# EmanuelOverflow/LSTM-TensorSpark

Measured on NVIDIA H100. Metric: samples/sec, higher is better.
Workload: dtype bf16

## Files before the change

### lstm_tensorspark_b200/csrc/bindings.cpp

```cpp
#include <torch/extension.h>
#include <ATen/cuda/CUDAContext.h>
#include <c10/cuda/CUDAGuard.h>
#include <c10/cuda/CUDAException.h>
#include <cuda_runtime.h>

#include <cmath>
#include <optional>
#include <string>
#include <vector>

using torch::Tensor;

extern "C" {
int ts_lstm_pointwise_fwd(const void*, const float*, const float*, void*, float*, void*, int, int, int, cudaStream_t, const void*,
                          const int*, int);
int ts_transpose01_rows(const void*, void*, int, int, long long, cudaStream_t);
int ts_lstm_seq_cluster_probe(int);
int ts_lstm_seq_config(int, int, int, int, int*);
int ts_transpose2d_b16(const void*, void*, int, int, cudaStream_t);
int ts_colsum_bf16(const void*, float*, void*, int, int, int, int, int, int, cudaStream_t);
long long ts_colsum_scratch_bytes(int, int);
int ts_lstm_pointwise_bwd(const void*, const float*, const float*, const void*, const float*, const float*, void*,
                          float*, int, int, int, cudaStream_t, const int*, int, float*);
int ts_xent_rows(const float*, const long long*, float*, float*, int*, int, int, cudaStream_t);
int ts_flat_adam(float*, const float*, float*, float*, void*, long long, float, float, float, float, float, float,
                 cudaStream_t, int*, long long, const float*);
int ts_flat_sgd(float*, const float*, void*, long long, float, float, float, cudaStream_t, long long, const float*);
long long ts_flat_grad_norm_scratch(long long);
int ts_flat_grad_norm(const float*, const float*, long long, float, float, long long, float, double*, float*, cudaStream_t);
int ts_cast_bf16(const float*, void*, long long, cudaStream_t);
int ts_fused_allreduce(const unsigned long long*, unsigned long long, unsigned long long, unsigned long long, float*,
                       float*, unsigned int*, int*, long long, int, int, int, int, int, int, float, float, float, float,
                       float, double, cudaStream_t, int*, long long, int, int);
int ts_ar_bump_step(int*, cudaStream_t);
int ts_ar_max_blocks();
int ts_ar_flag_words();
int ts_ar_slots();
int ts_head_fwd_tc(const void*, int, const float*, const float*, const long long*, float*, float*, float*, int*, int, int, int, cudaStream_t);
int ts_head_logits_generic(const void*, const float*, const float*, float*, int, int, int, int, cudaStream_t);
int ts_head_bwd(const void*, const float*, const float*, const float*, void*, float*, float*, int, int, int, int, int, cudaStream_t);
int ts_head_step_fwd_generic_parts(int);
int ts_head_step_fwd(const void*, int, int, const float*, const float*, const long long*, const int*, float*, float*, float*, int*,
                     unsigned int*, float*, int*, int*, int, int, int, int, int*, cudaStream_t);
long long ts_head_step_bwd_scratch(int, int, int);
int ts_head_step_bwd_tickets(int);
int ts_head_step_bwd(const void*, const float*, const float*, const float*, void*, float*, float*, float*, unsigned int*, int, int, int,
                     int, int, cudaStream_t);
int ts_vocab_head_parts(int);
int ts_vocab_head_blocks(int);
int ts_vocab_head_fwd(const void*, const void*, int, const float*, const long long*, const int*, void*, float*, float*, int*, unsigned int*,
                      float*, int*, int*, int, int, int, int, int, cudaStream_t);
int ts_vocab_head_dlogits(const void*, const void*, int, const float*, const long long*, const int*, const float*, const float*, const int*,
                          void*, int, int, int, int, int, int, int, cudaStream_t);
int ts_vocab_head_colsum(const void*, float*, int, int, int, cudaStream_t);
int ts_vocab_sample(const void*, const void*, int, const float*, float, unsigned int, int*, const int*, void*, int*, unsigned int*, int*,
                    float*, int*, float*, int, int, int, int, int, int, cudaStream_t);
int ts_vocab_sample_logits(const float*, const float*, float, unsigned int, int*, const int*, void*, int*, unsigned int*, int*, float*, int*,
                           float*, int, int, int, int, cudaStream_t);
int ts_vocab_head_logits(const void*, const void*, int, const float*, float*, int, int, int, int, cudaStream_t);
int ts_vocab_threshold(const float*, int, int, int, double, float, float*, cudaStream_t);
int ts_gemm_generic(const void*, const void*, void*, const float*, int, int, int, long long, long long, long long, long long, long long,
                    int, int, int, float, cudaStream_t);
int ts_gemm2(const void*, const void*, void*, const float*, int, int, int, int, int, int, int, int, int, int, int, int, int,
             const unsigned int*, const int*, unsigned int*, int*, int, int, int, int, float*, int, cudaStream_t);
int ts_lstm_seq_fwd(const void*, const void*, const float*, const void*, const float*, void*, const float*, void*, void*, int,
                    int, int, unsigned int*, int, cudaStream_t, const void*, const unsigned int*, int, int, int, const int*, int,
                    void*, const int*, const unsigned int*);
int ts_lstm_seq_bwd(const void*, const void*, const void*, const float*, const void*, float*, float*, void*, void*, int,
                    int, int, unsigned int*, int, cudaStream_t, const unsigned int*, int, int, int, const int*, int,
                    const int*, const unsigned int*);
int ts_dropout(const void*, void*, int, int, int, int, int, const int*, const unsigned int*, cudaStream_t);
int ts_lstm_seq_prologue(const void*, const float*, void*, float*, void*, unsigned int*, int, int, cudaStream_t);
int ts_seq_pool_fwd(const void*, int, const int*, const float*, int, int, int, int, float*, int*, cudaStream_t);
int ts_seq_pool_attn_scores(float*, const float*, const float*, const int*, int, int, int, float*, cudaStream_t);
int ts_seq_pool_attn_bwd(const void*, int, const float*, const float*, const float*, const float*, const int*, int, int, int, int,
                         float*, void*, float*, unsigned int*, float*, float*, int, int, cudaStream_t);
int ts_seq_pool_bwd(const float*, const int*, const int*, const float*, const float*, int, int, int, int, void*, int, cudaStream_t);
void ts_embed_scratch_numel(long long, long long, long long, long long*);
int ts_embed_fwd(const void*, int, const int*, const int*, int, int, int, int, void*, cudaStream_t);
int ts_embed_bwd(const void*, int, const int*, const int*, int, int, int, int, float*, int, int*, int*, float*, cudaStream_t);
int ts_embed_bwd_launches();
const char* ts_last_error();
}

namespace {

void check(int rc, const char* what) {
  if (rc != 0) {
    std::string msg = std::string(what) + " failed: rc=" + std::to_string(rc);
    if (rc > 0) msg += std::string(" (") + cudaGetErrorString((cudaError_t)rc) + ")";
    const char* le = ts_last_error();
    if (le && le[0]) msg += std::string(" [") + le + "]";
    TORCH_CHECK(false, msg);
  }
}
cudaStream_t stream() { return at::cuda::getCurrentCUDAStream().stream(); }
void chk_cuda(const Tensor& t, const char* n) {
  TORCH_CHECK(t.is_cuda(), n, " must be a CUDA tensor");
  TORCH_CHECK(t.is_contiguous(), n, " must be contiguous");
}
int is_bf16(const Tensor& t) {
  TORCH_CHECK(t.scalar_type() == torch::kBFloat16 || t.scalar_type() == torch::kFloat32, "dtype must be bf16 or fp32");
  return t.scalar_type() == torch::kBFloat16 ? 1 : 0;
}
const float* fptr(const std::optional<Tensor>& t) { return t.has_value() ? t->data_ptr<float>() : nullptr; }
const int* lengths_ptr(const std::optional<Tensor>& lengths, int64_t B, const Tensor& like) {
  if (!lengths.has_value()) return nullptr;
  const Tensor& l = *lengths;
  TORCH_CHECK(l.is_cuda() && l.device() == like.device(), "lengths must be on the batch's device");
  TORCH_CHECK(l.scalar_type() == torch::kInt32, "lengths must be int32");
  TORCH_CHECK(l.dim() == 1 && l.size(0) == B, "lengths must be [B] (B = ", B, ")");
  TORCH_CHECK(l.is_contiguous(), "lengths must be contiguous");
  return l.data_ptr<int>();
}
const int* drop_args(const std::optional<Tensor>& step, const std::vector<int64_t>& desc, const Tensor& like, unsigned int (&out)[5]) {
  if (!step.has_value()) return nullptr;
  TORCH_CHECK(step->is_cuda() && step->device() == like.device() && step->scalar_type() == torch::kInt32 && step->numel() == 1,
              "dropout: the step counter must be an int32 [1] tensor on the batch's device");
  TORCH_CHECK(desc.size() == 5, "dropout: desc = {key0, key1, thr, c2, row0}");
  TORCH_CHECK(desc[2] >= 1 && desc[2] <= 65535 && desc[4] >= 0, "dropout: thr in [1, 65535], row0 >= 0");
  for (int i = 0; i < 5; ++i) out[i] = (unsigned int)(uint32_t)desc[i];
  return step->data_ptr<int>();
}

int direction_flag(bool reverse, const std::optional<Tensor>& in_gate, bool extra_signal) {
  TORCH_CHECK(!reverse || (!in_gate.has_value() && !extra_signal), "reverse: the layer wavefront (in_gate / extra_signal) is forward-only");
  return reverse ? 1 : 0;
}

Tensor transpose01(const Tensor& x) {
  chk_cuda(x, "x");
  TORCH_CHECK(x.dim() == 3 && x.is_contiguous(), "transpose01: expected a contiguous [B,T,D] tensor");
  c10::cuda::CUDAGuard g(x.device());
  const int B = x.size(0), T = x.size(1);
  const long long row_bytes = (long long)x.size(2) * x.element_size();
  TORCH_CHECK(row_bytes % 16 == 0, "transpose01: row size must be a multiple of 16 bytes");
  auto out = torch::empty({x.size(1), x.size(0), x.size(2)}, x.options());
  check(ts_transpose01_rows(x.data_ptr(), out.data_ptr(), B, T, row_bytes, stream()), "transpose01");
  return out;
}

Tensor transpose2d(const Tensor& x) {
  chk_cuda(x, "x");
  TORCH_CHECK(x.dim() == 2 && x.is_contiguous() && x.element_size() == 2, "transpose2d: expected a contiguous 2-D 16-bit tensor");
  c10::cuda::CUDAGuard g(x.device());
  auto out = torch::empty({x.size(1), x.size(0)}, x.options());
  check(ts_transpose2d_b16(x.data_ptr(), out.data_ptr(), (int)x.size(0), (int)x.size(1), stream()), "transpose2d");
  return out;
}

void* colsum_scratch(const Tensor& x) {
  static std::vector<Tensor> bufs(64);
  const int dev = x.device().index();
  const int64_t need = ts_colsum_scratch_bytes((int)x.size(0), (int)x.size(1));
  if (!bufs[dev].defined() || bufs[dev].numel() < need)
    bufs[dev] = torch::zeros({need}, torch::TensorOptions().device(x.device()).dtype(torch::kUInt8));
  return bufs[dev].data_ptr();
}

Tensor colsum_bf16(const Tensor& x) {
  chk_cuda(x, "x");
  TORCH_CHECK(x.dim() == 2 && x.is_contiguous() && is_bf16(x) && x.size(1) % 256 == 0, "colsum_bf16: contiguous bf16 [rows, cols], cols % 256 == 0");
  c10::cuda::CUDAGuard g(x.device());
  auto out = torch::empty({x.size(1)}, x.options().dtype(torch::kFloat32));
  check(ts_colsum_bf16(x.data_ptr(), out.data_ptr<float>(), colsum_scratch(x), (int)x.size(0), (int)x.size(1), (int)x.size(1), 0, 0, 0, stream()), "colsum_bf16");
  return out;
}

void colsum_bf16_into(const Tensor& x, Tensor out, bool overwrite, bool pdl, int64_t col0, int64_t ncols, int64_t max_ctas) {
  chk_cuda(x, "x"); chk_cuda(out, "out");
  TORCH_CHECK(x.dim() == 2 && is_bf16(x) && x.size(1) % 256 == 0 && out.scalar_type() == torch::kFloat32 && out.numel() == x.size(1),
              "colsum_bf16_into: bf16 [rows, cols % 256 == 0] -> fp32 [cols]");
  if (ncols <= 0) { col0 = 0; ncols = x.size(1); }
  TORCH_CHECK(col0 % 256 == 0 && ncols % 256 == 0 && col0 + ncols <= x.size(1), "colsum_bf16_into: 256-aligned column range");
  c10::cuda::CUDAGuard g(x.device());
  check(ts_colsum_bf16((const char*)x.data_ptr() + 2 * col0, out.data_ptr<float>() + col0, colsum_scratch(x), (int)x.size(0), (int)ncols,
                       (int)x.size(1), overwrite ? 0 : 1, pdl ? 1 : 0, (int)max_ctas, stream()), "colsum_bf16_into");
}

std::vector<Tensor> lstm_pointwise_fwd(const Tensor& pre, const Tensor& bias, const Tensor& c_prev, const std::optional<Tensor>& h_prev,
                                       const std::optional<Tensor>& lengths, int64_t t) {
  chk_cuda(pre, "pre"); chk_cuda(bias, "bias"); chk_cuda(c_prev, "c_prev");
  c10::cuda::CUDAGuard g(pre.device());
  int B = pre.size(0), H = pre.size(1) / 4;
  TORCH_CHECK(bias.scalar_type() == torch::kFloat32 && c_prev.scalar_type() == torch::kFloat32, "bias/c must be fp32");
  TORCH_CHECK(c_prev.numel() == (int64_t)B * H && bias.numel() == 4 * H, "shape mismatch");
  const int* lp = lengths_ptr(lengths, B, pre);
  if (lp) {
    TORCH_CHECK(h_prev.has_value(), "lstm_pointwise_fwd: lengths need h_prev");
    chk_cuda(*h_prev, "h_prev");
    TORCH_CHECK(h_prev->scalar_type() == pre.scalar_type() && h_prev->numel() == (int64_t)B * H, "h_prev: [B,H] in pre's dtype");
  }
  auto h = torch::empty({B, H}, pre.options());
  auto c = torch::empty({B, H}, c_prev.options());
  auto act = torch::empty_like(pre);
  check(ts_lstm_pointwise_fwd(pre.data_ptr(), bias.data_ptr<float>(), c_prev.data_ptr<float>(), h.data_ptr(),
                              c.data_ptr<float>(), act.data_ptr(), B, H, is_bf16(pre), stream(), lp ? h_prev->data_ptr() : nullptr,
                              lp, (int)t), "lstm_pointwise_fwd");
  return {h, c, act};
}

std::vector<Tensor> lstm_pointwise_bwd(const std::optional<Tensor>& dh_a, const std::optional<Tensor>& dh_b,
                                       const std::optional<Tensor>& dc_in, const Tensor& act, const Tensor& c_prev,
                                       const Tensor& c_new, const std::optional<Tensor>& lengths, int64_t t) {
  chk_cuda(act, "act"); chk_cuda(c_prev, "c_prev"); chk_cuda(c_new, "c_new");
  c10::cuda::CUDAGuard g(act.device());
  int B = act.size(0), H = act.size(1) / 4;
  const int* lp = lengths_ptr(lengths, B, act);
  if (dh_a.has_value()) { chk_cuda(*dh_a, "dh_a"); TORCH_CHECK(dh_a->scalar_type() == act.scalar_type(), "dh_a dtype"); }
  if (dh_b.has_value()) { chk_cuda(*dh_b, "dh_b"); TORCH_CHECK(dh_b->scalar_type() == torch::kFloat32, "dh_b fp32"); }
  if (dc_in.has_value()) { chk_cuda(*dc_in, "dc_in"); TORCH_CHECK(dc_in->scalar_type() == torch::kFloat32, "dc fp32"); }
  auto dpre = torch::empty_like(act);
  auto dc = torch::empty_like(c_prev);
  Tensor dh_out = lp ? torch::empty_like(c_prev) : Tensor();
  check(ts_lstm_pointwise_bwd(dh_a.has_value() ? dh_a->data_ptr() : nullptr, fptr(dh_b), fptr(dc_in), act.data_ptr(),
                              c_prev.data_ptr<float>(), c_new.data_ptr<float>(), dpre.data_ptr(), dc.data_ptr<float>(),
                              B, H, is_bf16(act), stream(), lp, (int)t, lp ? dh_out.data_ptr<float>() : nullptr), "lstm_pointwise_bwd");
  if (lp) return {dpre, dc, dh_out};
  return {dpre, dc};
}

Tensor dropout(const Tensor& x, const Tensor& step, const std::vector<int64_t>& desc, int64_t t0) {
  chk_cuda(x, "x");
  TORCH_CHECK(x.dim() >= 2, "dropout: x must be [..., B, H]");
  c10::cuda::CUDAGuard g(x.device());
  unsigned int dd[5];
  const int* ds = drop_args(step, desc, x, dd);
  const int64_t B = x.size(-2), H = x.size(-1), steps = B * H ? x.numel() / (B * H) : 0;
  auto y = torch::empty_like(x);
  check(ts_dropout(x.data_ptr(), y.data_ptr(), (int)steps, (int)B, (int)H, (int)t0, is_bf16(x), ds, dd, stream()), "dropout");
  return y;
}

std::vector<Tensor> xent_rows(const Tensor& logits, const Tensor& labels) {
  chk_cuda(logits, "logits"); chk_cuda(labels, "labels");
  c10::cuda::CUDAGuard g(logits.device());
  TORCH_CHECK(logits.scalar_type() == torch::kFloat32 && labels.scalar_type() == torch::kInt64, "dtypes");
  int B = logits.size(0), C = logits.size(1);
  auto dlogits = torch::empty_like(logits);
  auto loss = torch::zeros({1}, logits.options());
  auto correct = torch::zeros({1}, logits.options().dtype(torch::kInt32));
  check(ts_xent_rows(logits.data_ptr<float>(), (const long long*)labels.data_ptr<int64_t>(), dlogits.data_ptr<float>(),
                     loss.data_ptr<float>(), correct.data_ptr<int>(), B, C, stream()), "xent_rows");
  return {dlogits, loss, correct};
}

std::vector<Tensor> head_fwd(const Tensor& h, const Tensor& W, const Tensor& bias, const Tensor& labels) {
  TORCH_CHECK(h.is_cuda() && h.dim() == 2 && h.stride(1) == 1, "head_fwd: h [B,H] with unit inner stride");
  chk_cuda(W, "W"); chk_cuda(bias, "bias"); chk_cuda(labels, "labels");
  c10::cuda::CUDAGuard g(h.device());
  const int B = h.size(0), H = h.size(1), C = W.size(1);
  TORCH_CHECK(W.size(0) == H && W.scalar_type() == torch::kFloat32 && bias.scalar_type() == torch::kFloat32, "head W/b");
  TORCH_CHECK(labels.scalar_type() == torch::kInt64 && labels.numel() == B, "labels int64 [B]");
  auto fo = torch::TensorOptions().device(h.device()).dtype(torch::kFloat32);
  auto logits = torch::empty({B, C}, fo), dlogits = torch::empty({B, C}, fo);
  auto loss = torch::zeros({1}, fo);
  auto correct = torch::zeros({1}, fo.dtype(torch::kInt32));
  int rc = -1;
  if (h.scalar_type() == torch::kBFloat16)
    rc = ts_head_fwd_tc(h.data_ptr(), (int)h.stride(0), W.data_ptr<float>(), bias.data_ptr<float>(), (const long long*)labels.data_ptr<int64_t>(),
                        logits.data_ptr<float>(), dlogits.data_ptr<float>(), loss.data_ptr<float>(), correct.data_ptr<int>(), B, H, C, stream());
  if (rc == -1) {
    auto hc = h.contiguous();
    check(ts_head_logits_generic(hc.data_ptr(), W.data_ptr<float>(), bias.data_ptr<float>(), logits.data_ptr<float>(), B, H, C, is_bf16(hc), stream()),
          "head_logits_generic");
    check(ts_xent_rows(logits.data_ptr<float>(), (const long long*)labels.data_ptr<int64_t>(), dlogits.data_ptr<float>(),
                       loss.data_ptr<float>(), correct.data_ptr<int>(), B, C, stream()), "xent_rows");
  } else {
    check(rc, "head_fwd_tc");
  }
  return {logits, dlogits, loss, correct};
}

Tensor head_bwd(const Tensor& h, const Tensor& W, const Tensor& dlogits, const std::optional<Tensor>& dloss, Tensor dW, Tensor db,
                bool accumulate) {
  chk_cuda(h, "h"); chk_cuda(W, "W"); chk_cuda(dlogits, "dlogits"); chk_cuda(dW, "dW"); chk_cuda(db, "db");
  c10::cuda::CUDAGuard g(h.device());
  const int B = h.size(0), H = h.size(1), C = W.size(1);
  TORCH_CHECK(dW.scalar_type() == torch::kFloat32 && db.scalar_type() == torch::kFloat32 && dW.numel() == (int64_t)H * C && db.numel() == C, "head_bwd: dW/db");
  TORCH_CHECK(dlogits.scalar_type() == torch::kFloat32 && dlogits.numel() == (int64_t)B * C, "head_bwd: dlogits fp32 [B,C]");
  auto dh = torch::empty_like(h);
  check(ts_head_bwd(h.data_ptr(), W.data_ptr<float>(), dlogits.data_ptr<float>(), fptr(dloss), dh.data_ptr(), dW.data_ptr<float>(),
                    db.data_ptr<float>(), B, H, C, is_bf16(h), accumulate ? 1 : 0, stream()), "head_bwd");
  return dh;
}

std::vector<Tensor> head_step_fwd(const Tensor& h, const Tensor& W, const Tensor& bias, const Tensor& labels,
                                  const std::optional<Tensor>& lengths, int64_t T) {
  TORCH_CHECK(h.is_cuda() && h.dim() == 2 && h.stride(1) == 1, "head_step_fwd: h [T*B,H] with unit inner stride");
  chk_cuda(W, "W"); chk_cuda(bias, "bias"); chk_cuda(labels, "labels");
  c10::cuda::CUDAGuard g(h.device());
  const int R = h.size(0), H = h.size(1), C = W.size(1);
  TORCH_CHECK(T >= 1 && R % T == 0, "head_step_fwd: rows must be T*B");
  const int B = R / (int)T;
  TORCH_CHECK(W.size(0) == H && W.scalar_type() == torch::kFloat32 && bias.scalar_type() == torch::kFloat32 && bias.numel() == C, "head W/b");
  TORCH_CHECK(labels.scalar_type() == torch::kInt64 && labels.dim() == 2 && labels.size(0) == B && labels.size(1) == T, "labels int64 [B,T]");
  const int* lp = nullptr;
  if (lengths.has_value()) {
    chk_cuda(*lengths, "lengths");
    TORCH_CHECK(lengths->scalar_type() == torch::kInt32 && lengths->numel() == B, "lengths int32 [B]");
    lp = lengths->data_ptr<int>();
  }
  auto fo = torch::TensorOptions().device(h.device()).dtype(torch::kFloat32);
  auto io = fo.dtype(torch::kInt32);
  auto logits = torch::empty({B, (int64_t)T, C}, fo), dlogits = torch::empty({R, C}, fo);
  const int parts = ts_head_step_fwd_generic_parts(R);
  auto part_loss = torch::empty({parts}, fo);
  auto ints = torch::zeros({parts + 4}, io);
  auto loss = torch::empty({1}, fo);
  Tensor hc = h;
  if (h.scalar_type() != torch::kBFloat16 && h.stride(0) != H) hc = h.contiguous();
  int used_tc = 0;
  int rc = ts_head_step_fwd(hc.data_ptr(), (int)hc.stride(0), is_bf16(hc), W.data_ptr<float>(), bias.data_ptr<float>(),
                            (const long long*)labels.data_ptr<int64_t>(), lp, logits.data_ptr<float>(), dlogits.data_ptr<float>(),
                            part_loss.data_ptr<float>(), ints.data_ptr<int>(), (unsigned int*)(ints.data_ptr<int>() + parts),
                            loss.data_ptr<float>(), ints.data_ptr<int>() + parts + 1, ints.data_ptr<int>() + parts + 2, (int)T, B, H, C,
                            &used_tc, stream());
  if (rc == -2) {
    hc = h.contiguous();
    rc = ts_head_step_fwd(hc.data_ptr(), H, 1, W.data_ptr<float>(), bias.data_ptr<float>(), (const long long*)labels.data_ptr<int64_t>(),
                          lp, logits.data_ptr<float>(), dlogits.data_ptr<float>(), part_loss.data_ptr<float>(), ints.data_ptr<int>(),
                          (unsigned int*)(ints.data_ptr<int>() + parts), loss.data_ptr<float>(), ints.data_ptr<int>() + parts + 1,
                          ints.data_ptr<int>() + parts + 2, (int)T, B, H, C, &used_tc, stream());
  }
  check(rc, "head_step_fwd");
  return {logits, dlogits, loss, ints.narrow(0, parts + 1, 1), ints.narrow(0, parts + 2, 1),
          torch::full({1}, used_tc, torch::TensorOptions().dtype(torch::kInt32))};
}

Tensor head_step_bwd(const Tensor& h, const Tensor& W, const Tensor& dlogits, const std::optional<Tensor>& dloss, Tensor dW, Tensor db,
                     bool accumulate) {
  chk_cuda(h, "h"); chk_cuda(W, "W"); chk_cuda(dlogits, "dlogits"); chk_cuda(dW, "dW"); chk_cuda(db, "db");
  c10::cuda::CUDAGuard g(h.device());
  const int R = h.size(0), H = h.size(1), C = W.size(1);
  TORCH_CHECK(dW.scalar_type() == torch::kFloat32 && db.scalar_type() == torch::kFloat32 && dW.numel() == (int64_t)H * C && db.numel() == C, "head_step_bwd: dW/db");
  TORCH_CHECK(dlogits.scalar_type() == torch::kFloat32 && dlogits.numel() == (int64_t)R * C, "head_step_bwd: dlogits fp32 [R,C]");
  auto dh = torch::empty_like(h);
  auto fo = torch::TensorOptions().device(h.device()).dtype(torch::kFloat32);
  auto scratch = torch::empty({std::max<long long>(1, ts_head_step_bwd_scratch(R, H, C))}, fo);
  auto tickets = torch::zeros({ts_head_step_bwd_tickets(H)}, fo.dtype(torch::kInt32));
  check(ts_head_step_bwd(h.data_ptr(), W.data_ptr<float>(), dlogits.data_ptr<float>(), fptr(dloss), dh.data_ptr(), dW.data_ptr<float>(),
                         db.data_ptr<float>(), scratch.data_ptr<float>(), (unsigned int*)tickets.data_ptr<int>(), R, H, C, is_bf16(h),
                         accumulate ? 1 : 0, stream()), "head_step_bwd");
  return dh;
}

int64_t vocab_classes(const Tensor& h, const Tensor& Wb, bool w_kmajor, const char* what) {
  TORCH_CHECK(h.dim() == 2 && Wb.dim() == 2 && h.scalar_type() == torch::kBFloat16 && Wb.scalar_type() == torch::kBFloat16 &&
              Wb.size(w_kmajor ? 1 : 0) == h.size(1), what, ": h bf16 [rows,H], Wb bf16 ", w_kmajor ? "[C,H]" : "[H,C]");
  TORCH_CHECK(!w_kmajor || (Wb.is_contiguous() && (uintptr_t)Wb.data_ptr() % 16 == 0), what, ": the table [C,H] must be packed and "
              "16-byte aligned (TMA)");
  return Wb.size(w_kmajor ? 0 : 1);
}

void vocab_head_check(const Tensor& h, const Tensor& Wb, bool w_kmajor, const Tensor& bias, const Tensor& labels, int64_t T) {
  chk_cuda(h, "h"); chk_cuda(Wb, "Wb"); chk_cuda(bias, "bias"); chk_cuda(labels, "labels");
  const int64_t R = h.size(0), H = h.size(1), C = vocab_classes(h, Wb, w_kmajor, "vocab head");
  TORCH_CHECK(H % 64 == 0 && C % 8 == 0 && C >= 8, "vocab head: H % 64 == 0 and C % 8 == 0");
  TORCH_CHECK(T >= 1 && R % T == 0 && R * std::max(C, H) < (int64_t(1) << 40) && R < (int64_t(1) << 31), "vocab head: rows must be T*B");
  TORCH_CHECK(bias.scalar_type() == torch::kFloat32 && bias.numel() == C && ((uintptr_t)bias.data_ptr() % 8) == 0, "vocab head: bias fp32 [C]");
  TORCH_CHECK(labels.scalar_type() == torch::kInt64 && labels.dim() == 2 && labels.size(0) == R / T && labels.size(1) == T, "labels int64 [B,T]");
}

std::vector<Tensor> vocab_head_fwd(const Tensor& h, const Tensor& Wb, bool w_kmajor, const Tensor& bias, const Tensor& labels,
                                   const std::optional<Tensor>& lengths, int64_t T, Tensor part) {
  vocab_head_check(h, Wb, w_kmajor, bias, labels, T);
  c10::cuda::CUDAGuard g(h.device());
  const int R = h.size(0), H = h.size(1), C = Wb.size(w_kmajor ? 0 : 1), B = R / (int)T;
  chk_cuda(part, "part");
  TORCH_CHECK(part.scalar_type() == torch::kFloat32 && part.numel() >= (int64_t)R * ts_vocab_head_parts(C) * 4 &&
              ((uintptr_t)part.data_ptr() % 16) == 0, "vocab head: part scratch");
  auto fo = torch::TensorOptions().device(h.device()).dtype(torch::kFloat32);
  const int blocks = ts_vocab_head_blocks(R);
  auto lse = torch::empty({R}, fo), part_loss = torch::empty({blocks}, fo), loss = torch::empty({1}, fo);
  auto ints = torch::zeros({blocks + 4}, fo.dtype(torch::kInt32));
  int* ip = ints.data_ptr<int>();
  check(ts_vocab_head_fwd(h.data_ptr(), Wb.data_ptr(), w_kmajor ? 1 : 0, bias.data_ptr<float>(), (const long long*)labels.data_ptr<int64_t>(),
                          lengths_ptr(lengths, B, h), part.data_ptr(), lse.data_ptr<float>(), part_loss.data_ptr<float>(), ip,
                          (unsigned int*)(ip + blocks), loss.data_ptr<float>(), ip + blocks + 1, ip + blocks + 2, (int)T, B, H, C,
                          h.get_device(), stream()), "vocab_head_fwd");
  return {lse, loss, ints.narrow(0, blocks + 1, 1), ints.narrow(0, blocks + 2, 1)};
}

void vocab_head_dlogits(const Tensor& h, const Tensor& Wb, bool w_kmajor, const Tensor& bias, const Tensor& labels,
                        const std::optional<Tensor>& lengths, int64_t T, const Tensor& lse, const Tensor& count, const Tensor& dloss,
                        int64_t row0, int64_t rows, Tensor dl) {
  vocab_head_check(h, Wb, w_kmajor, bias, labels, T);
  c10::cuda::CUDAGuard g(h.device());
  const int R = h.size(0), H = h.size(1), C = Wb.size(w_kmajor ? 0 : 1), B = R / (int)T;
  chk_cuda(lse, "lse"); chk_cuda(count, "count"); chk_cuda(dloss, "dloss"); chk_cuda(dl, "dl");
  TORCH_CHECK(lse.scalar_type() == torch::kFloat32 && lse.numel() == R && count.scalar_type() == torch::kInt32 && count.numel() == 1 &&
              dloss.scalar_type() == torch::kFloat32 && dloss.numel() == 1, "vocab head: lse fp32 [R], count int32 [1], dloss fp32 [1]");
  TORCH_CHECK(rows >= 1 && row0 >= 0 && row0 + rows <= R && dl.scalar_type() == torch::kBFloat16 && dl.numel() >= rows * C,
              "vocab head: dl bf16 [rows, C]");
  check(ts_vocab_head_dlogits(h.data_ptr(), Wb.data_ptr(), w_kmajor ? 1 : 0, bias.data_ptr<float>(), (const long long*)labels.data_ptr<int64_t>(),
                              lengths_ptr(lengths, B, h), lse.data_ptr<float>(), dloss.data_ptr<float>(), count.data_ptr<int>(),
                              dl.data_ptr(), (int)T, B, H, C, (int)row0, (int)rows, h.get_device(), stream()), "vocab_head_dlogits");
}

void vocab_head_colsum(const Tensor& dl, Tensor db, bool accumulate) {
  chk_cuda(dl, "dl"); chk_cuda(db, "db");
  c10::cuda::CUDAGuard g(dl.device());
  TORCH_CHECK(dl.dim() == 2 && dl.scalar_type() == torch::kBFloat16 && dl.size(1) % 2 == 0 && db.scalar_type() == torch::kFloat32 &&
              db.numel() == dl.size(1), "vocab head: dl bf16 [rows, C], db fp32 [C]");
  check(ts_vocab_head_colsum(dl.data_ptr(), db.data_ptr<float>(), (int)dl.size(0), (int)dl.size(1), accumulate ? 1 : 0, stream()),
        "vocab_head_colsum");
}

struct SampleOut {
  int* rec_tok = nullptr;
  float* rec_lp = nullptr;
  int N = 0;
};
SampleOut sample_check(int64_t B, const Tensor& like, const Tensor& step, const Tensor& row0, const Tensor& tokens,
                       const std::optional<Tensor>& rec_tok, const std::optional<Tensor>& rec_lp, double temperature) {
  chk_cuda(step, "step"); chk_cuda(row0, "row0"); chk_cuda(tokens, "tokens");
  TORCH_CHECK(row0.scalar_type() == torch::kInt32 && row0.numel() == 1 && row0.device() == like.device(), "vocab sample: row0 int32 [1]");
  TORCH_CHECK(std::isfinite(temperature) && temperature >= 0, "vocab sample: temperature must be finite and >= 0");
  TORCH_CHECK(step.scalar_type() == torch::kInt32 && step.numel() == 1 && step.device() == like.device(), "vocab sample: step int32 [1]");
  TORCH_CHECK(tokens.scalar_type() == torch::kInt32 && tokens.numel() == B && tokens.device() == like.device(), "vocab sample: tokens int32 [B]");
  SampleOut o;
  TORCH_CHECK(rec_tok.has_value() == rec_lp.has_value(), "vocab sample: rec_tok and rec_lp go together");
  if (rec_tok.has_value()) {
    chk_cuda(*rec_tok, "rec_tok"); chk_cuda(*rec_lp, "rec_lp");
    TORCH_CHECK(rec_tok->scalar_type() == torch::kInt32 && rec_tok->dim() == 2 && rec_tok->size(0) == B &&
                rec_lp->scalar_type() == torch::kFloat32 && rec_lp->sizes() == rec_tok->sizes() &&
                rec_tok->device() == like.device() && rec_lp->device() == like.device(), "vocab sample: records int32 / fp32 [B, N]");
    o.rec_tok = rec_tok->data_ptr<int>(); o.rec_lp = rec_lp->data_ptr<float>(); o.N = (int)rec_tok->size(1);
  }
  return o;
}

Tensor vocab_sample(const Tensor& h, const Tensor& Wb, bool w_kmajor, const Tensor& bias, double temperature, int64_t seed, Tensor step,
                    const Tensor& row0, Tensor tokens, const std::optional<Tensor>& rec_tok, const std::optional<Tensor>& rec_lp,
                    int64_t s0) {
  chk_cuda(h, "h"); chk_cuda(Wb, "Wb"); chk_cuda(bias, "bias");
  const int64_t Cw = vocab_classes(h, Wb, w_kmajor, "vocab sample");
  TORCH_CHECK(h.size(0) >= 1 && h.size(0) < (int64_t(1) << 24), "vocab sample: h bf16 [B,H] with 1 <= B < 2^24");
  TORCH_CHECK(h.size(1) % 64 == 0 && Cw % 8 == 0 && Cw >= 8, "vocab sample: H % 64 == 0 and C % 8 == 0");
  TORCH_CHECK(bias.scalar_type() == torch::kFloat32 && bias.numel() == Cw && ((uintptr_t)bias.data_ptr() % 8) == 0,
              "vocab sample: bias fp32 [C]");
  c10::cuda::CUDAGuard g(h.device());
  const int B = h.size(0), H = h.size(1), C = (int)Cw;
  const SampleOut o = sample_check(B, h, step, row0, tokens, rec_tok, rec_lp, temperature);
  const int nt = ts_vocab_head_parts(C);
  auto fo = torch::TensorOptions().device(h.device()).dtype(torch::kFloat32);
  auto part = torch::empty({(int64_t)B * nt * 4}, fo), logprob = torch::empty({B}, fo);
  auto part_arg = torch::empty({(int64_t)B * nt}, fo.dtype(torch::kInt32)), ticket = torch::zeros({1}, fo.dtype(torch::kInt32));
  check(ts_vocab_sample(h.data_ptr(), Wb.data_ptr(), w_kmajor ? 1 : 0, bias.data_ptr<float>(), (float)temperature, (unsigned int)(seed & 0xffffffff),
                        step.data_ptr<int>(), row0.data_ptr<int>(), part.data_ptr(), part_arg.data_ptr<int>(), (unsigned int*)ticket.data_ptr<int>(),
                        tokens.data_ptr<int>(), logprob.data_ptr<float>(), o.rec_tok, o.rec_lp, o.N, (int)s0, B, H, C, h.get_device(),
                        stream()), "vocab_sample");
  return logprob;
}

void chk_logits(const Tensor& logits) {
  chk_cuda(logits, "logits");
  TORCH_CHECK(logits.dim() == 2 && logits.scalar_type() == torch::kFloat32 && logits.is_contiguous() && logits.size(0) >= 1 &&
              logits.size(1) >= 1 && logits.size(1) < (int64_t(1) << 31) && logits.numel() < (int64_t(1) << 40),
              "vocab sample: logits fp32 [B, C], packed");
}

Tensor vocab_sample_logits(const Tensor& logits, double temperature, int64_t seed, Tensor step, const Tensor& row0, Tensor tokens,
                           const std::optional<Tensor>& rec_tok, const std::optional<Tensor>& rec_lp, int64_t s0,
                           const std::optional<Tensor>& tau) {
  chk_logits(logits);
  c10::cuda::CUDAGuard g(logits.device());
  const int B = logits.size(0), C = logits.size(1);
  const SampleOut o = sample_check(B, logits, step, row0, tokens, rec_tok, rec_lp, temperature);
  if (tau.has_value()) {
    chk_cuda(*tau, "tau");
    TORCH_CHECK(tau->scalar_type() == torch::kFloat32 && tau->numel() == B && tau->is_contiguous() && tau->device() == logits.device(),
                "vocab sample: tau fp32 [B]");
    TORCH_CHECK(temperature > 0, "vocab sample: a threshold needs temperature > 0 (greedy keeps the arg-max, which no filter drops)");
  }
  const int nt = ts_vocab_head_parts(C);
  auto fo = torch::TensorOptions().device(logits.device()).dtype(torch::kFloat32);
  auto part = torch::empty({(int64_t)B * nt * 4}, fo), logprob = torch::empty({B}, fo);
  auto part_arg = torch::empty({(int64_t)B * nt}, fo.dtype(torch::kInt32)), ticket = torch::zeros({1}, fo.dtype(torch::kInt32));
  check(ts_vocab_sample_logits(logits.data_ptr<float>(), tau.has_value() ? tau->data_ptr<float>() : nullptr, (float)temperature,
                               (unsigned int)(seed & 0xffffffff), step.data_ptr<int>(),
                               row0.data_ptr<int>(), part.data_ptr(), part_arg.data_ptr<int>(), (unsigned int*)ticket.data_ptr<int>(), tokens.data_ptr<int>(),
                               logprob.data_ptr<float>(), o.rec_tok, o.rec_lp, o.N, (int)s0, B, C, stream()), "vocab_sample_logits");
  return logprob;
}

Tensor vocab_head_logits(const Tensor& h, const Tensor& Wb, bool w_kmajor, const Tensor& bias) {
  chk_cuda(h, "h"); chk_cuda(Wb, "Wb"); chk_cuda(bias, "bias");
  const int64_t Cw = vocab_classes(h, Wb, w_kmajor, "vocab logits");
  TORCH_CHECK(h.is_contiguous() && h.size(0) >= 1 && h.size(0) < (int64_t(1) << 24), "vocab logits: h bf16 [B,H] packed, 1 <= B < 2^24");
  TORCH_CHECK(h.size(1) % 64 == 0 && Cw % 8 == 0 && Cw >= 8, "vocab logits: H % 64 == 0 and C % 8 == 0");
  TORCH_CHECK(bias.scalar_type() == torch::kFloat32 && bias.numel() == Cw && ((uintptr_t)bias.data_ptr() % 8) == 0,
              "vocab logits: bias fp32 [C]");
  c10::cuda::CUDAGuard g(h.device());
  const int B = h.size(0), H = h.size(1), C = (int)Cw;
  auto logits = torch::empty({B, C}, torch::TensorOptions().device(h.device()).dtype(torch::kFloat32));
  check(ts_vocab_head_logits(h.data_ptr(), Wb.data_ptr(), w_kmajor ? 1 : 0, bias.data_ptr<float>(), logits.data_ptr<float>(), B, H, C,
                             h.get_device(), stream()), "vocab_head_logits");
  return logits;
}

Tensor vocab_threshold(const Tensor& logits, int64_t top_k, double top_p, double temperature) {
  chk_logits(logits);
  TORCH_CHECK(top_k >= 0, "vocab threshold: top_k must be >= 0 (0 = off), got ", top_k);
  TORCH_CHECK(std::isfinite(top_p) && top_p > 0 && top_p <= 1, "vocab threshold: top_p must be in (0, 1] (1 = off), got ", top_p);
  TORCH_CHECK(std::isfinite(temperature) && temperature > 0, "vocab threshold: temperature must be finite and > 0, got ", temperature);
  c10::cuda::CUDAGuard g(logits.device());
  const int B = logits.size(0), C = logits.size(1);
  auto tau = torch::empty({B}, torch::TensorOptions().device(logits.device()).dtype(torch::kFloat32));
  check(ts_vocab_threshold(logits.data_ptr<float>(), B, C, (int)std::min<int64_t>(top_k, C), top_p, (float)temperature,
                           tau.data_ptr<float>(), stream()), "vocab_threshold");
  return tau;
}

void chk_f32(const Tensor& t, int64_t numel, const char* n) {
  chk_cuda(t, n);
  TORCH_CHECK(t.scalar_type() == torch::kFloat32 && t.numel() == numel, n, ": fp32 with ", numel, " elements");
}

std::vector<Tensor> seq_pool_fwd(const Tensor& h, const std::optional<Tensor>& lengths, int64_t T, int64_t mode,
                                 const std::optional<Tensor>& alpha) {
  chk_cuda(h, "h");
  TORCH_CHECK(h.dim() == 2 && T >= 1 && h.size(0) % T == 0, "seq_pool_fwd: h [T·B, H]");
  TORCH_CHECK(mode >= 0 && mode <= 2, "seq_pool_fwd: mode 0 mean, 1 max, 2 attention");
  c10::cuda::CUDAGuard g(h.device());
  const int B = h.size(0) / T, H = h.size(1);
  if (mode == 2) {
    TORCH_CHECK(alpha.has_value(), "seq_pool_fwd: attention needs alpha");
    chk_f32(*alpha, (int64_t)T * B, "alpha");
  }
  auto fo = h.options().dtype(torch::kFloat32);
  auto s = torch::empty({B, H}, fo);
  auto am = mode == 1 ? torch::empty({B, H}, fo.dtype(torch::kInt32)) : torch::empty({0}, fo.dtype(torch::kInt32));
  check(ts_seq_pool_fwd(h.data_ptr(), is_bf16(h), lengths_ptr(lengths, B, h), fptr(alpha), (int)mode, (int)T, B, H,
                        s.data_ptr<float>(), mode == 1 ? am.data_ptr<int>() : nullptr, stream()), "seq_pool_fwd");
  return {s, am};
}

Tensor seq_pool_attn_scores(Tensor u, const Tensor& ba, const Tensor& v, const std::optional<Tensor>& lengths, int64_t T) {
  chk_cuda(u, "u");
  TORCH_CHECK(u.dim() == 2 && u.scalar_type() == torch::kFloat32 && T >= 1 && u.size(0) % T == 0, "seq_pool_attn_scores: u fp32 [T·B, A]");
  c10::cuda::CUDAGuard g(u.device());
  const int B = u.size(0) / T, A = u.size(1);
  chk_f32(ba, A, "b_a"); chk_f32(v, A, "v");
  auto alpha = torch::empty({T, B}, u.options());
  check(ts_seq_pool_attn_scores(u.data_ptr<float>(), ba.data_ptr<float>(), v.data_ptr<float>(), lengths_ptr(lengths, B, u), (int)T, B, A,
                                alpha.data_ptr<float>(), stream()), "seq_pool_attn_scores");
  return alpha;
}

Tensor seq_pool_attn_bwd(const Tensor& h, const Tensor& ds, const Tensor& alpha, const Tensor& u, const Tensor& v,
                         const std::optional<Tensor>& lengths, int64_t T, Tensor dv, Tensor dba, bool acc_dv, bool acc_dba) {
  chk_cuda(h, "h");
  TORCH_CHECK(h.dim() == 2 && T >= 1 && h.size(0) % T == 0, "seq_pool_attn_bwd: h [T·B, H]");
  c10::cuda::CUDAGuard g(h.device());
  const int B = h.size(0) / T, H = h.size(1), A = u.size(1);
  chk_f32(ds, (int64_t)B * H, "ds"); chk_f32(alpha, (int64_t)T * B, "alpha"); chk_f32(u, (int64_t)T * B * A, "u");
  chk_f32(v, A, "v"); chk_f32(dv, A, "dv"); chk_f32(dba, A, "dba");
  auto fo = h.options().dtype(torch::kFloat32);
  auto dU = torch::empty({h.size(0), A}, h.options());
  auto dalpha = torch::empty({T, B}, fo);
  auto partial = torch::empty({B, 2 * A}, fo);
  auto ticket = torch::zeros({1}, fo.dtype(torch::kInt32));
  check(ts_seq_pool_attn_bwd(h.data_ptr(), is_bf16(h), ds.data_ptr<float>(), alpha.data_ptr<float>(), u.data_ptr<float>(),
                             v.data_ptr<float>(), lengths_ptr(lengths, B, h), (int)T, B, H, A, dalpha.data_ptr<float>(), dU.data_ptr(),
                             partial.data_ptr<float>(), (unsigned int*)ticket.data_ptr<int>(), dv.data_ptr<float>(), dba.data_ptr<float>(),
                             acc_dv ? 1 : 0, acc_dba ? 1 : 0, stream()), "seq_pool_attn_bwd");
  return dU;
}

Tensor seq_pool_bwd(const Tensor& ds, const std::optional<Tensor>& lengths, int64_t T, int64_t mode, const std::optional<Tensor>& argmax,
                    const std::optional<Tensor>& alpha, const std::optional<Tensor>& G, bool out_bf16) {
  chk_cuda(ds, "ds");
  TORCH_CHECK(ds.dim() == 2 && ds.scalar_type() == torch::kFloat32 && T >= 1, "seq_pool_bwd: ds fp32 [B,H]");
  TORCH_CHECK(mode >= 0 && mode <= 2, "seq_pool_bwd: mode 0 mean, 1 max, 2 attention");
  c10::cuda::CUDAGuard g(ds.device());
  const int B = ds.size(0), H = ds.size(1);
  if (mode == 1) {
    TORCH_CHECK(argmax.has_value() && argmax->scalar_type() == torch::kInt32 && argmax->numel() == (int64_t)B * H, "seq_pool_bwd: argmax int32 [B,H]");
    chk_cuda(*argmax, "argmax");
  }
  if (mode == 2) {
    TORCH_CHECK(alpha.has_value() && G.has_value(), "seq_pool_bwd: attention needs alpha and G");
    chk_f32(*alpha, (int64_t)T * B, "alpha"); chk_f32(*G, (int64_t)T * B * H, "G");
  }
  auto dh = torch::empty({T * B, H}, ds.options().dtype(out_bf16 ? torch::kBFloat16 : torch::kFloat32));
  check(ts_seq_pool_bwd(ds.data_ptr<float>(), lengths_ptr(lengths, B, ds), mode == 1 ? argmax->data_ptr<int>() : nullptr, fptr(alpha),
                        fptr(G), (int)mode, (int)T, B, H, dh.data_ptr(), out_bf16 ? 1 : 0, stream()), "seq_pool_bwd");
  return dh;
}

void chk_tokens(const Tensor& tok, const Tensor& like) {
  chk_cuda(tok, "tokens");
  TORCH_CHECK(tok.device() == like.device() && tok.scalar_type() == torch::kInt32 && tok.dim() == 2,
              "tokens must be int32 [B,T] on the table's device");
}

Tensor embed_fwd(const Tensor& table, const Tensor& tokens, const std::optional<Tensor>& lengths) {
  chk_cuda(table, "table");
  TORCH_CHECK(table.dim() == 2, "embed_fwd: table [V,E]");
  chk_tokens(tokens, table);
  c10::cuda::CUDAGuard g(table.device());
  const int B = tokens.size(0), T = tokens.size(1), V = table.size(0), E = table.size(1);
  auto x = torch::empty({T, B, E}, table.options());
  check(ts_embed_fwd(table.data_ptr(), is_bf16(table), tokens.data_ptr<int>(), lengths_ptr(lengths, B, table), T, B, E, V,
                     x.data_ptr(), stream()), "embed_fwd");
  return x;
}

struct EmbedScratch { int* zeroed; int* ints; float* floats; };
EmbedScratch embed_scratch(const Tensor& like, int64_t N, int64_t V, int64_t E) {
  static std::vector<std::vector<Tensor>> bufs(64, std::vector<Tensor>(3));
  static std::vector<Tensor> retired;
  auto& b = bufs[like.device().index()];
  long long need[2];
  ts_embed_scratch_numel(N, V, E, need);
  const int64_t sizes[3] = {2 * V, need[0], need[1]};
  for (int i = 0; i < 3; ++i) {
    if (b[i].defined() && b[i].numel() >= sizes[i]) continue;
    if (b[i].defined()) retired.push_back(b[i]);
    auto opt = torch::TensorOptions().device(like.device()).dtype(i == 2 ? torch::kFloat32 : torch::kInt32);
    b[i] = i == 0 ? torch::zeros({sizes[i]}, opt) : torch::empty({sizes[i]}, opt);
  }
  return {b[0].data_ptr<int>(), b[1].data_ptr<int>(), b[2].data_ptr<float>()};
}

void embed_bwd(const Tensor& dx, const Tensor& tokens, const std::optional<Tensor>& lengths, Tensor dW, bool accumulate) {
  chk_cuda(dx, "dx"); chk_cuda(dW, "dW");
  chk_tokens(tokens, dx);
  const int B = tokens.size(0), T = tokens.size(1);
  TORCH_CHECK(dW.dim() == 2 && dW.scalar_type() == torch::kFloat32 && dW.device() == dx.device(), "embed_bwd: dW fp32 [V,E]");
  const int V = dW.size(0), E = dW.size(1);
  TORCH_CHECK(dx.numel() == (int64_t)T * B * E, "embed_bwd: dx [T·B, E]");
  c10::cuda::CUDAGuard g(dx.device());
  auto s = embed_scratch(dx, (int64_t)T * B, V, E);
  check(ts_embed_bwd(dx.data_ptr(), is_bf16(dx), tokens.data_ptr<int>(), lengths_ptr(lengths, B, dx), T, B, E, V,
                     dW.data_ptr<float>(), accumulate ? 1 : 0, s.zeroed, s.ints, s.floats, stream()), "embed_bwd");
}

const float* clip_ptr(const std::optional<Tensor>& clip, const Tensor& p) {
  if (!clip.has_value()) return nullptr;
  TORCH_CHECK(clip->is_cuda() && clip->device() == p.device() && clip->scalar_type() == torch::kFloat32 && clip->numel() == 2 &&
              clip->is_contiguous(), "clip must be a contiguous fp32 [2] tensor on p's device (flat_grad_norm's out)");
  return clip->data_ptr<float>();
}
void flat_adam(Tensor p, const Tensor& g, Tensor m, Tensor v, std::optional<Tensor> shadow, double lr_t, double b1,
               double b2, double eps, double wd, double gscale, std::optional<Tensor> step_dev, int64_t wd_numel,
               std::optional<Tensor> clip) {
  chk_cuda(p, "p"); chk_cuda(g, "g"); chk_cuda(m, "m"); chk_cuda(v, "v");
  c10::cuda::CUDAGuard gd(p.device());
  TORCH_CHECK(p.numel() == g.numel() && p.numel() == m.numel() && p.numel() == v.numel(), "numel mismatch");
  check(ts_flat_adam(p.data_ptr<float>(), g.data_ptr<float>(), m.data_ptr<float>(), v.data_ptr<float>(),
                     shadow.has_value() ? shadow->data_ptr() : nullptr, p.numel(), lr_t, b1, b2, eps, wd, gscale, stream(),
                     step_dev.has_value() ? step_dev->data_ptr<int>() : nullptr, (long long)wd_numel, clip_ptr(clip, p)),
        "flat_adam");
}
void flat_sgd(Tensor p, const Tensor& g, std::optional<Tensor> shadow, double lr, double wd, double gscale, int64_t wd_numel,
              std::optional<Tensor> clip) {
  chk_cuda(p, "p"); chk_cuda(g, "g");
  c10::cuda::CUDAGuard gd(p.device());
  check(ts_flat_sgd(p.data_ptr<float>(), g.data_ptr<float>(), shadow.has_value() ? shadow->data_ptr() : nullptr,
                    p.numel(), lr, wd, gscale, stream(), (long long)wd_numel, clip_ptr(clip, p)), "flat_sgd");
}
void flat_grad_norm(const Tensor& g, const Tensor& p, Tensor out, Tensor scratch, double max_norm, double wd, double gscale,
                    int64_t wd_numel) {
  chk_cuda(g, "g"); chk_cuda(p, "p"); chk_cuda(out, "out"); chk_cuda(scratch, "scratch");
  c10::cuda::CUDAGuard gd(g.device());
  TORCH_CHECK(g.scalar_type() == torch::kFloat32 && p.scalar_type() == torch::kFloat32 && p.numel() == g.numel(), "flat_grad_norm: g, p fp32 of one size");
  TORCH_CHECK(out.scalar_type() == torch::kFloat32 && out.numel() == 2, "flat_grad_norm: out fp32 [2]");
  TORCH_CHECK(scratch.scalar_type() == torch::kFloat64 && scratch.numel() >= ts_flat_grad_norm_scratch(g.numel()),
              "flat_grad_norm: scratch float64 [flat_grad_norm_scratch(n)]");
  TORCH_CHECK(p.device() == g.device() && out.device() == g.device() && scratch.device() == g.device(), "flat_grad_norm: one device");
  check(ts_flat_grad_norm(g.data_ptr<float>(), p.data_ptr<float>(), g.numel(), wd, gscale, (long long)wd_numel, max_norm,
                          scratch.data_ptr<double>(), out.data_ptr<float>(), stream()), "flat_grad_norm");
}
void cast_bf16(const Tensor& p, Tensor shadow) {
  chk_cuda(p, "p"); chk_cuda(shadow, "shadow");
  c10::cuda::CUDAGuard gd(p.device());
  TORCH_CHECK(shadow.scalar_type() == torch::kBFloat16 && shadow.numel() == p.numel(), "shadow");
  check(ts_cast_bf16(p.data_ptr<float>(), shadow.data_ptr(), p.numel(), stream()), "cast_bf16");
}

void fused_allreduce(const Tensor& ptrs, int64_t mc_in, int64_t mc_param, int64_t mc_shadow, std::optional<Tensor> m,
                     std::optional<Tensor> v, Tensor epochs, Tensor err, int64_t n, int64_t rank, int64_t world,
                     int64_t mode, bool two_shot, bool multicast, int64_t blocks, double lr, double b1, double b2,
                     double eps, double wd, double timeout_s, std::optional<Tensor> step_dev, int64_t wd_numel, bool bump_step, bool pdl) {
  TORCH_CHECK(!ptrs.is_cuda() && ptrs.scalar_type() == torch::kInt64 && ptrs.numel() == 4 * world, "ptrs: cpu int64 [4,world]");
  chk_cuda(epochs, "epochs"); chk_cuda(err, "err");
  c10::cuda::CUDAGuard gd(epochs.device());
  check(ts_fused_allreduce((const unsigned long long*)ptrs.data_ptr<int64_t>(), (unsigned long long)mc_in,
                           (unsigned long long)mc_param, (unsigned long long)mc_shadow,
                           m.has_value() ? m->data_ptr<float>() : nullptr, v.has_value() ? v->data_ptr<float>() : nullptr,
                           (unsigned int*)epochs.data_ptr<int>(), err.data_ptr<int>(), n, (int)rank, (int)world, (int)mode,
                           two_shot ? 1 : 0, multicast ? 1 : 0, (int)blocks, lr, b1, b2, eps, wd, timeout_s, stream(),
                           step_dev.has_value() ? step_dev->data_ptr<int>() : nullptr, (long long)wd_numel, bump_step ? 1 : 0, pdl ? 1 : 0),
        "fused_allreduce");
}

Tensor gemm2(const Tensor& A, const Tensor& B, const std::optional<Tensor>& bias, std::optional<Tensor> out, bool a_mn, bool b_mn,
             bool out_fp32, bool accumulate, int64_t ctas, int64_t bn, int64_t max_ctas, const std::optional<Tensor>& gate,
             const std::vector<int64_t>& gate_cfg, const std::optional<Tensor>& done, const std::optional<Tensor>& gate_err,
             int64_t stream_handle, bool pdl, int64_t a_fold, int64_t b_fold, int64_t fold_cols, const std::optional<Tensor>& rowsum,
             bool rowsum_acc) {
  TORCH_CHECK(A.is_cuda() && B.is_cuda(), "gemm2: CUDA tensors");
  TORCH_CHECK(!(a_fold && b_fold) && (!a_fold || !a_mn) && (!b_fold || b_mn), "gemm2: one folded operand (K-major A or MN-major B)");
  TORCH_CHECK(A.scalar_type() == torch::kBFloat16 && B.scalar_type() == torch::kBFloat16, "gemm2: A/B must be bf16");
  TORCH_CHECK(A.dim() == 2 && B.dim() == 2 && A.stride(1) == 1 && B.stride(1) == 1, "gemm2: 2-D operands with unit inner stride");
  c10::cuda::CUDAGuard gd(A.device());
  if (a_fold) TORCH_CHECK(A.size(0) == a_fold && fold_cols > 0 && A.size(1) % fold_cols == 0, "gemm2: folded A must be [fold, T * fold_cols]");
  if (b_fold) TORCH_CHECK(B.size(0) == b_fold && fold_cols > 0 && B.size(1) % fold_cols == 0, "gemm2: folded B must be [fold, T * fold_cols]");
  const int M = a_fold ? (int)(a_fold * (A.size(1) / fold_cols)) : (a_mn ? A.size(1) : A.size(0));
  const int K = a_fold ? (int)fold_cols : (a_mn ? A.size(0) : A.size(1));
  const int N = b_fold ? (int)fold_cols : (b_mn ? B.size(1) : B.size(0));
  const int Kb = b_fold ? (int)(b_fold * (B.size(1) / fold_cols)) : (b_mn ? B.size(0) : B.size(1));
  TORCH_CHECK(K == Kb, "gemm2: contraction sizes differ (", K, " vs ", Kb, ")");
  Tensor C;
  if (out.has_value()) {
    C = *out;
    TORCH_CHECK(C.is_cuda() && C.dim() == 2 && C.size(0) == M && C.size(1) == N && C.stride(1) == 1, "gemm2: out must be [M,N]");
    TORCH_CHECK(C.scalar_type() == (out_fp32 || accumulate ? torch::kFloat32 : torch::kBFloat16), "gemm2: out dtype");
  } else {
    TORCH_CHECK(!accumulate, "gemm2: accumulate needs out=");
    C = torch::empty({M, N}, A.options().dtype(out_fp32 ? torch::kFloat32 : torch::kBFloat16));
  }
  const int out_mode = accumulate ? 2 : (C.scalar_type() == torch::kFloat32 ? 1 : 0);
  const unsigned int* gp = nullptr;
  int gcfg[7] = {0, 0, 0, 0, 1, 0, 0};
  if (gate.has_value()) {
    TORCH_CHECK(gate->is_cuda() && gate->scalar_type() == torch::kInt32 && gate_cfg.size() == 7, "gemm2: gate int32 cuda + 7 config ints");
    gp = (const unsigned int*)gate->data_ptr<int>();
    for (int i = 0; i < 7; ++i) gcfg[i] = (int)gate_cfg[i];
  }
  float* rp = nullptr;
  if (rowsum.has_value()) {
    TORCH_CHECK(rowsum->is_cuda() && rowsum->scalar_type() == torch::kFloat32 && rowsum->is_contiguous() && rowsum->numel() == M &&
                C.scalar_type() == torch::kFloat32, "gemm2: rowsum must be a contiguous fp32 [M] next to an fp32 output");
    rp = rowsum->data_ptr<float>();
  }
  TORCH_CHECK((ctas == 1 || ctas == 2) && (bn == 128 || bn == 256), "gemm2: ctas must be 1 or 2 and bn 128 or 256 (got ", ctas, ", ", bn, ")");
  unsigned int* dp = nullptr;
  if (done.has_value()) {
    TORCH_CHECK(done->is_cuda() && done->scalar_type() == torch::kInt32 && done->is_contiguous(), "gemm2: done must be a contiguous int32 cuda tensor");
    const int64_t blocks = (M + 128 * ctas - 1) / (128 * ctas) * ctas * ((N + bn - 1) / bn);
    TORCH_CHECK(done->numel() >= blocks, "gemm2: done needs ceil(M / (128 * ctas)) * ctas * ceil(N / bn) = ", blocks,
                " counters, got ", done->numel());
    dp = (unsigned int*)done->data_ptr<int>();
  }
  check(ts_gemm2(A.data_ptr(), B.data_ptr(), C.data_ptr(), fptr(bias), M, N, K, (int)A.stride(0), (int)B.stride(0), (int)C.stride(0),
                 a_mn ? 1 : 0, b_mn ? 1 : 0, out_mode, (int)ctas, (int)bn, A.device().index(), (int)max_ctas, gp, gcfg, dp,
                 gate_err.has_value() ? gate_err->data_ptr<int>() : nullptr, pdl ? 1 : 0, (int)a_fold, (int)b_fold, (int)fold_cols,
                 rp, rowsum_acc ? 1 : 0, stream_handle ? (cudaStream_t)stream_handle : stream()), "gemm2");
  return C;
}

Tensor gemm_generic(const Tensor& A, const Tensor& B, const std::optional<Tensor>& bias, std::optional<Tensor> out, bool out_fp32, double beta) {
  TORCH_CHECK(A.is_cuda() && B.is_cuda() && A.dim() == 2 && B.dim() == 2 && A.size(1) == B.size(0), "gemm_generic: A [M,K] x B [K,N]");
  c10::cuda::CUDAGuard gd(A.device());
  const int M = A.size(0), K = A.size(1), N = B.size(1);
  Tensor C;
  if (out.has_value()) {
    C = *out;
    TORCH_CHECK(C.is_cuda() && C.dim() == 2 && C.size(0) == M && C.size(1) == N && C.stride(1) == 1, "gemm_generic: out [M,N]");
  } else {
    TORCH_CHECK(beta == 0.0, "gemm_generic: beta needs out=");
    C = torch::empty({M, N}, A.options().dtype(out_fp32 ? torch::kFloat32 : A.scalar_type()));
  }
  check(ts_gemm_generic(A.data_ptr(), B.data_ptr(), C.data_ptr(), fptr(bias), M, N, K, A.stride(0), A.stride(1), B.stride(0), B.stride(1),
                        C.stride(0), is_bf16(A), is_bf16(B), is_bf16(C), (float)beta, stream()), "gemm_generic");
  return C;
}

std::vector<Tensor> lstm_seq_fwd(const Tensor& gx, const Tensor& w_h, const Tensor& bias, const Tensor& h0,
                                 const Tensor& c0, Tensor sync_ws, int64_t variant, std::optional<Tensor> dbg,
                                 std::optional<Tensor> in_gate, int64_t in_gate_tiles_n, bool extra_signal,
                                 const std::optional<Tensor>& lengths, bool reverse, const std::optional<Tensor>& drop_step,
                                 const std::vector<int64_t>& drop_desc) {
  chk_cuda(gx, "gx"); chk_cuda(w_h, "w_h"); chk_cuda(bias, "bias"); chk_cuda(h0, "h0"); chk_cuda(c0, "c0");
  c10::cuda::CUDAGuard gd(gx.device());
  int T = gx.size(0), B = gx.size(1), H = gx.size(2) / 4;
  const int* lp = lengths_ptr(lengths, B, gx);
  const int rev = direction_flag(reverse, in_gate, extra_signal);
  unsigned int dd[5];
  const int* ds = drop_args(drop_step, drop_desc, gx, dd);
  Tensor h_drop = ds ? torch::empty({T, B, H}, gx.options()) : Tensor();
  auto h_seq = torch::empty({T + 1, B, H}, gx.options());
  auto c_seq = torch::empty({T + 1, B, H}, c0.options());
  auto act = torch::empty({T, B, 4 * H}, gx.options());
  const int tiles_m = (B + 127) / 128, nkb = H / 64;
  auto tiled = torch::empty({(int64_t)(T + 1), tiles_m, nkb, 128, 64}, gx.options());
  TORCH_CHECK(h0.scalar_type() == torch::kBFloat16 && c0.scalar_type() == torch::kFloat32, "h0 bf16 / c0 fp32");
  check(ts_lstm_seq_fwd(gx.data_ptr(), w_h.data_ptr(), bias.data_ptr<float>(), h_seq.data_ptr(), c_seq.data_ptr<float>(),
                        act.data_ptr(), c0.data_ptr<float>(), dbg.has_value() ? dbg->data_ptr() : nullptr, tiled.data_ptr(), T, B, H,
                        (unsigned int*)sync_ws.data_ptr<int>(), (int)variant, stream(), h0.data_ptr(),
                        in_gate.has_value() ? (const unsigned int*)in_gate->data_ptr<int>() : nullptr, (int)in_gate_tiles_n,
                        extra_signal ? 1 : 0, 0, lp, rev, ds ? h_drop.data_ptr() : nullptr, ds, dd), "lstm_seq_fwd");
  if (ds) return {h_seq, c_seq, act, h_drop};
  return {h_seq, c_seq, act};
}

std::vector<Tensor> lstm_seq_bwd(const std::optional<Tensor>& dh_seq, const Tensor& w_hT, const Tensor& act, const Tensor& c_seq,
                                 const Tensor& dhT, const Tensor& dcT, Tensor sync_ws, int64_t variant,
                                 std::optional<Tensor> dbg, std::optional<Tensor> in_gate, int64_t in_gate_tiles_n, bool extra_signal,
                                 const std::optional<Tensor>& lengths, bool reverse, const std::optional<Tensor>& drop_step,
                                 const std::vector<int64_t>& drop_desc) {
  if (dh_seq.has_value()) chk_cuda(*dh_seq, "dh_seq");
  chk_cuda(w_hT, "w_hT"); chk_cuda(act, "act"); chk_cuda(c_seq, "c_seq");
  c10::cuda::CUDAGuard gd(act.device());
  int T = act.size(0), B = act.size(1), H = act.size(2) / 4;
  const int* lp = lengths_ptr(lengths, B, act);
  const int rev = direction_flag(reverse, in_gate, extra_signal);
  unsigned int dd[5];
  const int* ds = drop_args(drop_step, drop_desc, act, dd);
  auto dpre = torch::empty_like(act);
  auto dh0 = dhT.clone();
  auto dc0 = dcT.clone();
  const int tiles_m = (B + 127) / 128;
  auto tiled = torch::empty({(int64_t)T, tiles_m, 4 * H / 64, 128, 64}, act.options());
  check(ts_lstm_seq_bwd(dh_seq.has_value() ? dh_seq->data_ptr() : nullptr, w_hT.data_ptr(), act.data_ptr(), c_seq.data_ptr<float>(), dpre.data_ptr(),
                        dh0.data_ptr<float>(), dc0.data_ptr<float>(), dbg.has_value() ? dbg->data_ptr() : nullptr, tiled.data_ptr(), T, B, H,
                        (unsigned int*)sync_ws.data_ptr<int>(), (int)variant, stream(),
                        in_gate.has_value() ? (const unsigned int*)in_gate->data_ptr<int>() : nullptr, (int)in_gate_tiles_n,
                        extra_signal ? 1 : 0, 0, lp, rev, ds, dd), "lstm_seq_bwd");
  return {dpre, dh0, dc0};
}

void lstm_seq_fwd_into(const Tensor& gx, const Tensor& w_h, const Tensor& bias, const Tensor& h0, const Tensor& c0, Tensor h_seq,
                       Tensor c_seq, Tensor act, Tensor tiled, Tensor sync_ws, int64_t variant, std::optional<Tensor> in_gate,
                       int64_t in_gate_tiles_n, bool extra_signal, int64_t stream_handle, int64_t launch_flags,
                       const std::optional<Tensor>& lengths, bool reverse, const std::optional<Tensor>& h_drop,
                       const std::optional<Tensor>& drop_step, const std::vector<int64_t>& drop_desc) {
  chk_cuda(gx, "gx"); chk_cuda(w_h, "w_h"); chk_cuda(bias, "bias"); chk_cuda(h0, "h0"); chk_cuda(c0, "c0");
  chk_cuda(h_seq, "h_seq"); chk_cuda(c_seq, "c_seq"); chk_cuda(act, "act"); chk_cuda(tiled, "tiled");
  c10::cuda::CUDAGuard gd(gx.device());
  int T = gx.size(0), B = gx.size(1), H = gx.size(2) / 4;
  const int* lp = lengths_ptr(lengths, B, gx);
  const int rev = direction_flag(reverse, in_gate, extra_signal);
  TORCH_CHECK(h_seq.numel() == (int64_t)(T + 1) * B * H && c_seq.numel() == h_seq.numel() && act.numel() == gx.numel(), "lstm_seq_fwd_into: buffer sizes");
  TORCH_CHECK(tiled.numel() == (int64_t)(T + 1) * ((B + 127) / 128) * 128 * H, "lstm_seq_fwd_into: tile-image buffer size");
  TORCH_CHECK(h0.scalar_type() == torch::kBFloat16 && c0.scalar_type() == torch::kFloat32, "h0 bf16 / c0 fp32");
  unsigned int dd[5];
  const int* ds = drop_args(drop_step, drop_desc, gx, dd);
  if (ds) {
    TORCH_CHECK(h_drop.has_value(), "lstm_seq_fwd_into: dropout needs h_drop");
    chk_cuda(*h_drop, "h_drop");
    TORCH_CHECK(h_drop->scalar_type() == gx.scalar_type() && h_drop->numel() == (int64_t)T * B * H, "lstm_seq_fwd_into: h_drop [T,B,H]");
  }
  check(ts_lstm_seq_fwd(gx.data_ptr(), w_h.data_ptr(), bias.data_ptr<float>(), h_seq.data_ptr(), c_seq.data_ptr<float>(),
                        act.data_ptr(), c0.data_ptr<float>(), nullptr, tiled.data_ptr(), T, B, H, (unsigned int*)sync_ws.data_ptr<int>(),
                        (int)variant, stream_handle ? (cudaStream_t)stream_handle : stream(), h0.data_ptr(),
                        in_gate.has_value() ? (const unsigned int*)in_gate->data_ptr<int>() : nullptr, (int)in_gate_tiles_n,
                        extra_signal ? 1 : 0, (int)launch_flags, lp, rev, ds ? h_drop->data_ptr() : nullptr, ds, dd), "lstm_seq_fwd_into");
}

void lstm_seq_prologue(const Tensor& h0, const Tensor& c0, Tensor h_seq, Tensor c_seq, Tensor tiled, Tensor sync_ws, bool reverse) {
  chk_cuda(h0, "h0"); chk_cuda(c0, "c0"); chk_cuda(h_seq, "h_seq"); chk_cuda(c_seq, "c_seq"); chk_cuda(tiled, "tiled");
  c10::cuda::CUDAGuard gd(h0.device());
  TORCH_CHECK(h0.scalar_type() == torch::kBFloat16 && c0.scalar_type() == torch::kFloat32 && h0.dim() == 2, "h0 bf16 [B,H] / c0 fp32");
  TORCH_CHECK(h_seq.scalar_type() == torch::kBFloat16 && h_seq.numel() % h0.numel() == 0 && h_seq.numel() >= h0.numel() &&
              c_seq.numel() == h_seq.numel(), "lstm_seq_prologue: h_seq bf16 / c_seq [T+1,B,H]");
  const int64_t init_off = reverse ? h_seq.numel() - h0.numel() : 0;
  check(ts_lstm_seq_prologue(h0.data_ptr(), c0.data_ptr<float>(), (at::BFloat16*)h_seq.data_ptr() + init_off, c_seq.data_ptr<float>() + init_off, tiled.data_ptr(),
                             (unsigned int*)sync_ws.data_ptr<int>(), (int)h0.size(0), (int)h0.size(1), stream()), "lstm_seq_prologue");
}

void lstm_seq_bwd_into(const std::optional<Tensor>& dh_seq, const Tensor& w_hT, const Tensor& act, const Tensor& c_seq, Tensor dpre,
                       Tensor dh0, Tensor dc0, Tensor tiled, Tensor sync_ws, int64_t variant, std::optional<Tensor> in_gate,
                       int64_t in_gate_tiles_n, bool extra_signal, int64_t stream_handle, int64_t launch_flags,
                       const std::optional<Tensor>& lengths, bool reverse, const std::optional<Tensor>& drop_step,
                       const std::vector<int64_t>& drop_desc) {
  chk_cuda(w_hT, "w_hT"); chk_cuda(act, "act"); chk_cuda(c_seq, "c_seq"); chk_cuda(dpre, "dpre"); chk_cuda(dh0, "dh0"); chk_cuda(dc0, "dc0");
  c10::cuda::CUDAGuard gd(act.device());
  int T = act.size(0), B = act.size(1), H = act.size(2) / 4;
  const int* lp = lengths_ptr(lengths, B, act);
  const int rev = direction_flag(reverse, in_gate, extra_signal);
  TORCH_CHECK(dpre.numel() == act.numel() && tiled.numel() == (int64_t)T * ((B + 127) / 128) * 128 * 4 * H, "lstm_seq_bwd_into: buffer sizes");
  TORCH_CHECK(dh0.scalar_type() == torch::kFloat32 && dc0.scalar_type() == torch::kFloat32 && dh0.numel() == (int64_t)B * H && dc0.numel() == (int64_t)B * H, "dh0/dc0 fp32 [B,H]");
  unsigned int dd[5];
  const int* ds = drop_args(drop_step, drop_desc, act, dd);
  check(ts_lstm_seq_bwd(dh_seq.has_value() ? dh_seq->data_ptr() : nullptr, w_hT.data_ptr(), act.data_ptr(), c_seq.data_ptr<float>(), dpre.data_ptr(),
                        dh0.data_ptr<float>(), dc0.data_ptr<float>(), nullptr, tiled.data_ptr(), T, B, H, (unsigned int*)sync_ws.data_ptr<int>(),
                        (int)variant, stream_handle ? (cudaStream_t)stream_handle : stream(),
                        in_gate.has_value() ? (const unsigned int*)in_gate->data_ptr<int>() : nullptr, (int)in_gate_tiles_n,
                        extra_signal ? 1 : 0, (int)launch_flags, lp, rev, ds, dd), "lstm_seq_bwd_into");
}

}

PYBIND11_MODULE(TORCH_EXTENSION_NAME, m) {
  m.doc() = "lstm_tensorspark_b200 sm_90a kernels";
  m.def("lstm_pointwise_fwd", &lstm_pointwise_fwd, py::arg("pre"), py::arg("bias"), py::arg("c_prev"), py::arg("h_prev") = py::none(),
        py::arg("lengths") = py::none(), py::arg("t") = 0);
  m.def("transpose01", &transpose01);
  m.def("transpose2d", &transpose2d);
  m.def("colsum_bf16", &colsum_bf16);
  m.def("colsum_bf16_into", &colsum_bf16_into, py::arg("x"), py::arg("out"), py::arg("overwrite"), py::arg("pdl") = false,
        py::arg("col0") = 0, py::arg("ncols") = 0, py::arg("max_ctas") = 0);
  m.def("lstm_seq_cluster_probe", [](int64_t c) { return ts_lstm_seq_cluster_probe((int)c); });
  m.def("lstm_seq_config", [](bool bwd, int64_t H, int64_t B, int64_t variant) {
    int out[4];
    check(ts_lstm_seq_config(bwd ? 1 : 0, (int)H, (int)B, (int)variant, out), "lstm_seq_config");
    return std::make_tuple(out[0], out[1], out[2] != 0, out[3] != 0);
  }, py::arg("bwd"), py::arg("H"), py::arg("B"), py::arg("variant") = 0);
  m.def("lstm_pointwise_bwd", &lstm_pointwise_bwd, py::arg("dh_a"), py::arg("dh_b"), py::arg("dc_in"), py::arg("act"), py::arg("c_prev"),
        py::arg("c_new"), py::arg("lengths") = py::none(), py::arg("t") = 0);
  m.def("xent_rows", &xent_rows);
  m.def("head_fwd", &head_fwd);
  m.def("seq_pool_fwd", &seq_pool_fwd, py::arg("h"), py::arg("lengths"), py::arg("T"), py::arg("mode"), py::arg("alpha"));
  m.def("seq_pool_attn_scores", &seq_pool_attn_scores, py::arg("u"), py::arg("b_a"), py::arg("v"), py::arg("lengths"), py::arg("T"));
  m.def("seq_pool_attn_bwd", &seq_pool_attn_bwd, py::arg("h"), py::arg("ds"), py::arg("alpha"), py::arg("u"), py::arg("v"),
        py::arg("lengths"), py::arg("T"), py::arg("dv"), py::arg("dba"), py::arg("acc_dv"), py::arg("acc_dba"));
  m.def("seq_pool_bwd", &seq_pool_bwd, py::arg("ds"), py::arg("lengths"), py::arg("T"), py::arg("mode"), py::arg("argmax"),
        py::arg("alpha"), py::arg("G"), py::arg("out_bf16"));
  m.def("embed_fwd", &embed_fwd, py::arg("table"), py::arg("tokens"), py::arg("lengths"));
  m.def("embed_bwd", &embed_bwd, py::arg("dx"), py::arg("tokens"), py::arg("lengths"), py::arg("dW"), py::arg("accumulate"));
  m.attr("EMBED_BWD_LAUNCHES") = ts_embed_bwd_launches();
  m.def("head_step_fwd", &head_step_fwd, py::arg("h"), py::arg("W"), py::arg("bias"), py::arg("labels"), py::arg("lengths"), py::arg("T"));
  m.def("head_step_bwd", &head_step_bwd, py::arg("h"), py::arg("W"), py::arg("dlogits"), py::arg("dloss"), py::arg("dW"), py::arg("db"),
        py::arg("accumulate"));
  m.def("vocab_head_parts", [](int64_t C) { return ts_vocab_head_parts((int)C); });
  m.def("vocab_head_fwd", &vocab_head_fwd, py::arg("h"), py::arg("Wb"), py::arg("w_kmajor"), py::arg("bias"), py::arg("labels"), py::arg("lengths"),
        py::arg("T"), py::arg("part"));
  m.def("vocab_head_dlogits", &vocab_head_dlogits, py::arg("h"), py::arg("Wb"), py::arg("w_kmajor"), py::arg("bias"), py::arg("labels"), py::arg("lengths"),
        py::arg("T"), py::arg("lse"), py::arg("count"), py::arg("dloss"), py::arg("row0"), py::arg("rows"), py::arg("dl"));
  m.def("vocab_head_colsum", &vocab_head_colsum, py::arg("dl"), py::arg("db"), py::arg("accumulate"));
  m.def("vocab_sample", &vocab_sample, py::arg("h"), py::arg("Wb"), py::arg("w_kmajor"), py::arg("bias"), py::arg("temperature"), py::arg("seed"),
        py::arg("step"), py::arg("row0"), py::arg("tokens"), py::arg("rec_tok"), py::arg("rec_lp"), py::arg("s0"));
  m.def("vocab_sample_logits", &vocab_sample_logits, py::arg("logits"), py::arg("temperature"), py::arg("seed"), py::arg("step"),
        py::arg("row0"), py::arg("tokens"), py::arg("rec_tok"), py::arg("rec_lp"), py::arg("s0"), py::arg("tau") = py::none());
  m.def("vocab_head_logits", &vocab_head_logits, py::arg("h"), py::arg("Wb"), py::arg("w_kmajor"), py::arg("bias"));
  m.def("vocab_threshold", &vocab_threshold, py::arg("logits"), py::arg("top_k"), py::arg("top_p"), py::arg("temperature"));
  m.def("head_bwd", &head_bwd, py::arg("h"), py::arg("W"), py::arg("dlogits"), py::arg("dloss"), py::arg("dW"), py::arg("db"),
        py::arg("accumulate") = false);
  m.def("flat_adam", &flat_adam, py::arg("p"), py::arg("g"), py::arg("m"), py::arg("v"), py::arg("shadow"), py::arg("lr_t"),
        py::arg("b1"), py::arg("b2"), py::arg("eps"), py::arg("wd"), py::arg("gscale"), py::arg("step_dev") = py::none(),
        py::arg("wd_numel") = -1, py::arg("clip") = py::none());
  m.def("flat_sgd", &flat_sgd, py::arg("p"), py::arg("g"), py::arg("shadow"), py::arg("lr"), py::arg("wd"), py::arg("gscale"),
        py::arg("wd_numel") = -1, py::arg("clip") = py::none());
  m.def("flat_grad_norm", &flat_grad_norm, py::arg("g"), py::arg("p"), py::arg("out"), py::arg("scratch"), py::arg("max_norm"),
        py::arg("wd") = 0.0, py::arg("gscale") = 1.0, py::arg("wd_numel") = -1);
  m.def("flat_grad_norm_scratch", [](int64_t n) { return ts_flat_grad_norm_scratch((long long)n); });
  m.def("cast_bf16", &cast_bf16);
  m.def("fused_allreduce", &fused_allreduce, py::arg("ptrs"), py::arg("mc_in"), py::arg("mc_param"), py::arg("mc_shadow"), py::arg("m"),
        py::arg("v"), py::arg("epochs"), py::arg("err"), py::arg("n"), py::arg("rank"), py::arg("world"), py::arg("mode"),
        py::arg("two_shot"), py::arg("multicast"), py::arg("blocks"), py::arg("lr"), py::arg("b1"), py::arg("b2"), py::arg("eps"),
        py::arg("wd"), py::arg("timeout_s"), py::arg("step_dev") = py::none(), py::arg("wd_numel") = -1, py::arg("bump_step") = true,
        py::arg("pdl") = false);
  m.def("ar_bump_step", [](Tensor step_dev) {
    TORCH_CHECK(step_dev.is_cuda() && step_dev.scalar_type() == torch::kInt32, "ar_bump_step: int32 cuda tensor");
    c10::cuda::CUDAGuard gd(step_dev.device());
    check(ts_ar_bump_step(step_dev.data_ptr<int>(), stream()), "ar_bump_step");
  });
  m.def("ar_max_blocks", []() { return ts_ar_max_blocks(); });
  m.def("ar_flag_words", []() { return ts_ar_flag_words(); });
  m.def("ar_slots", []() { return ts_ar_slots(); });
  m.def("gemm_generic", &gemm_generic, py::arg("A"), py::arg("B"), py::arg("bias") = py::none(), py::arg("out") = py::none(),
        py::arg("out_fp32") = false, py::arg("beta") = 0.0);
  m.def("gemm2", &gemm2, py::arg("A"), py::arg("B"), py::arg("bias") = py::none(), py::arg("out") = py::none(), py::arg("a_mn") = false,
        py::arg("b_mn") = false, py::arg("out_fp32") = false, py::arg("accumulate") = false, py::arg("ctas") = 2, py::arg("bn") = 256,
        py::arg("max_ctas") = 0, py::arg("gate") = py::none(), py::arg("gate_cfg") = std::vector<int64_t>{}, py::arg("done") = py::none(),
        py::arg("gate_err") = py::none(), py::arg("stream") = 0, py::arg("pdl") = false, py::arg("a_fold") = 0, py::arg("b_fold") = 0,
        py::arg("fold_cols") = 0, py::arg("rowsum") = py::none(), py::arg("rowsum_acc") = false);
  m.def("lstm_seq_fwd", &lstm_seq_fwd, py::arg("gx"), py::arg("w_h"), py::arg("bias"), py::arg("h0"), py::arg("c0"),
        py::arg("sync_ws"), py::arg("variant") = 0, py::arg("dbg") = py::none(), py::arg("in_gate") = py::none(),
        py::arg("in_gate_tiles_n") = 0, py::arg("extra_signal") = false, py::arg("lengths") = py::none(), py::arg("reverse") = false,
        py::arg("drop_step") = py::none(), py::arg("drop_desc") = std::vector<int64_t>{});
  m.def("lstm_seq_fwd_into", &lstm_seq_fwd_into, py::arg("gx"), py::arg("w_h"), py::arg("bias"), py::arg("h0"), py::arg("c0"),
        py::arg("h_seq"), py::arg("c_seq"), py::arg("act"), py::arg("tiled"), py::arg("sync_ws"), py::arg("variant"),
        py::arg("in_gate") = py::none(), py::arg("in_gate_tiles_n") = 0, py::arg("extra_signal") = false, py::arg("stream") = 0,
        py::arg("launch_flags") = 0, py::arg("lengths") = py::none(), py::arg("reverse") = false, py::arg("h_drop") = py::none(),
        py::arg("drop_step") = py::none(), py::arg("drop_desc") = std::vector<int64_t>{});
  m.def("lstm_seq_prologue", &lstm_seq_prologue, py::arg("h0"), py::arg("c0"), py::arg("h_seq"), py::arg("c_seq"), py::arg("tiled"),
        py::arg("sync_ws"), py::arg("reverse") = false);
  m.def("lstm_seq_bwd_into", &lstm_seq_bwd_into, py::arg("dh_seq"), py::arg("w_hT"), py::arg("act"), py::arg("c_seq"), py::arg("dpre"),
        py::arg("dh0"), py::arg("dc0"), py::arg("tiled"), py::arg("sync_ws"), py::arg("variant"), py::arg("in_gate") = py::none(),
        py::arg("in_gate_tiles_n") = 0, py::arg("extra_signal") = false, py::arg("stream") = 0, py::arg("launch_flags") = 0,
        py::arg("lengths") = py::none(), py::arg("reverse") = false, py::arg("drop_step") = py::none(),
        py::arg("drop_desc") = std::vector<int64_t>{});
  m.def("lstm_seq_bwd", &lstm_seq_bwd, py::arg("dh_seq"), py::arg("w_hT"), py::arg("act"), py::arg("c_seq"), py::arg("dhT"),
        py::arg("dcT"), py::arg("sync_ws"), py::arg("variant") = 0, py::arg("dbg") = py::none(), py::arg("in_gate") = py::none(),
        py::arg("in_gate_tiles_n") = 0, py::arg("extra_signal") = false, py::arg("lengths") = py::none(), py::arg("reverse") = false,
        py::arg("drop_step") = py::none(), py::arg("drop_desc") = std::vector<int64_t>{});
  m.def("dropout", &dropout, py::arg("x"), py::arg("step"), py::arg("desc"), py::arg("t0") = 0);
}
```

### lstm_tensorspark_b200/csrc/gemm2_wgmma.cu

```cuda
#include <cuda.h>
#include <cuda_bf16.h>
#include <cuda_runtime.h>
#include <stdio.h>
#include <string.h>

#include "hopper.cuh"
#include "tmap.h"

namespace {

constexpr int BM = 128;
constexpr int BK = 64;
constexpr int kThreads = 384;
constexpr int kConsWarp0 = 4;

enum OutMode { OUT_BF16 = 0, OUT_F32 = 1, OUT_F32_ACC = 2 };

template <int kCtas, int BN> struct Cfg2 {
  static constexpr int kBNCta = BN / kCtas;
  static constexpr int kABytes = BM * BK * 2;
  static constexpr int kBBytes = BN * BK * 2;
  static constexpr int kStageBytes = kABytes + kBBytes;
  static constexpr int kStages = (200 * 1024) / kStageBytes > 8 ? 8 : (200 * 1024) / kStageBytes;
  static constexpr int kSmemBytes = kStages * kStageBytes + 1024  + 1024
                                     + 1024 ;
};

TC_DEVICE uint32_t cluster_ctarank2() { uint32_t r; asm volatile("mov.u32 %0, %%cluster_ctarank;" : "=r"(r)); return r; }
TC_DEVICE void cluster_sync2() {
  asm volatile("barrier.cluster.arrive.release.aligned;" ::: "memory");
  asm volatile("barrier.cluster.wait.acquire.aligned;" ::: "memory");
}
TC_DEVICE uint32_t mapa2(uint32_t local_smem_addr, uint32_t cta) {
  uint32_t r;
  asm volatile("mapa.shared::cluster.u32 %0, %1, %2;" : "=r"(r) : "r"(local_smem_addr), "r"(cta));
  return r;
}
TC_DEVICE void mbar_arrive_cluster(uint32_t cluster_bar_addr) {
  asm volatile("mbarrier.arrive.release.cluster.shared::cluster.b64 _, [%0];" ::"r"(cluster_bar_addr) : "memory");
}

struct Gemm2Params {
  void* C;
  const float* bias;
  int M, N, K, ldc;
  const unsigned int* gate;
  int gate_count, gate_stride, gate_base, gate_per_step, gate_rows_per_step, gate_use_last;
  long long gate_spin_limit;
  int* gate_err;
  unsigned int* done;
  int pdl;
  int reverse_m;
  int a_fold, b_fold, fold_cols;
  float* rowsum;
  int rowsum_acc;
};

template <int kCtas, int BN, bool kAMN, bool kBMN, int kOut>
__global__ void __launch_bounds__(kThreads, 1)
gemm2_kernel(const __grid_constant__ CUtensorMap tmap_a, const __grid_constant__ CUtensorMap tmap_b, const Gemm2Params p) {
  using C = Cfg2<kCtas, BN>;
  extern __shared__ uint8_t smem_raw[];
  uint8_t* smem = reinterpret_cast<uint8_t*>((reinterpret_cast<uintptr_t>(smem_raw) + 1023) & ~uintptr_t(1023));
  uint8_t* smem_a = smem;
  uint8_t* smem_b = smem + C::kStages * C::kABytes;
  uint64_t* bars = reinterpret_cast<uint64_t*>(smem + C::kStages * C::kStageBytes);
  uint64_t* full = bars;
  uint64_t* empty = bars + C::kStages;
  uint8_t* smem_ones = smem + C::kStages * C::kStageBytes + 1024;

  const int warp = threadIdx.x >> 5;
  const int lane = threadIdx.x & 31;
  asm volatile("griddepcontrol.launch_dependents;" ::: "memory");
  const uint32_t crank = kCtas == 2 ? cluster_ctarank2() : 0u;
  constexpr int TM = BM * kCtas;
  const int tiles_n = (p.N + BN - 1) / BN;
  const int tiles_m = (p.M + TM - 1) / TM;
  const int num_tiles = tiles_m * tiles_n;
  const int num_kb = (p.K + BK - 1) / BK;
  const int cluster_id = blockIdx.x / kCtas, num_clusters = gridDim.x / kCtas;
  auto tile_m_of = [&](int tile) { const int tm = tile / tiles_n; return p.reverse_m ? tiles_m - 1 - tm : tm; };

  if (warp == 0 && lane == 0) {
    tc::prefetch_tmap(&tmap_a);
    tc::prefetch_tmap(&tmap_b);
  }
  if (warp == 1 && lane == 0) {
    for (int s = 0; s < C::kStages; ++s) { tc::mbar_init(&full[s], 1); tc::mbar_init(&empty[s], 8 * kCtas); }
    tc::fence_barrier_init();
  }
  __syncthreads();
  if (kCtas == 2) cluster_sync2();

  if (warp == 0) {
    const uint32_t full0 = tc::smem_u32(full), empty0 = tc::smem_u32(empty);
    const uint32_t sa0 = tc::smem_u32(smem_a), sb0 = tc::smem_u32(smem_b);
    uint32_t stage = 0, phase = 0;
    bool ok = true;
    int gate_t_ok = -1;
    bool gate_dead = false;
    for (int tile = cluster_id; tile < num_tiles && ok; tile += num_clusters) {
      const int m0 = tile_m_of(tile) * TM + (int)crank * BM;
      const int n0 = (tile % tiles_n) * BN + (int)crank * C::kBNCta;
      if (p.gate != nullptr) {
        const int r0 = tile_m_of(tile) * TM, r1 = min(r0 + TM, p.M) - 1;
        const int t = (p.gate_use_last ? r1 : r0) / p.gate_rows_per_step;
        if (t != gate_t_ok && !gate_dead) {
          const int target = p.gate_base + p.gate_per_step * t;
          const long long t0 = clock64();
          for (int g = lane; g < p.gate_count; g += 32) {
            const unsigned int* c = p.gate + (size_t)g * p.gate_stride;
            unsigned int v;
            while (true) {
              asm volatile("ld.relaxed.gpu.global.u32 %0, [%1];" : "=r"(v) : "l"(c) : "memory");
              if ((int)v - target >= 0) break;
              if (clock64() - t0 > p.gate_spin_limit) { if (p.gate_err) atomicExch(p.gate_err, 1); ok = false; break; }
            }
          }
          ok = __all_sync(0xffffffffu, ok);
          asm volatile("fence.acq_rel.gpu;" ::: "memory");
          asm volatile("fence.proxy.async.global;" ::: "memory");
          if (!ok) { gate_dead = true; ok = true; }
          gate_t_ok = t;
        }
      }
      const int a_col = (!kAMN && p.a_fold) ? (m0 / p.a_fold) * p.fold_cols : 0;
      const int a_row = (!kAMN && p.a_fold) ? m0 % p.a_fold : m0;
      for (int kb = 0, k0 = 0; kb < num_kb; ++kb, k0 += BK) {
        const uint32_t eb = empty0 + 8 * stage, fb = full0 + 8 * stage;
        while (!tc::mbar_try_wait_u32(eb, phase ^ 1)) {}
        if (tc::elect_one()) {
          tc::mbar_expect_tx_u32(fb, C::kStageBytes);
          const uint32_t sa = sa0 + stage * C::kABytes;
          const uint32_t sb = sb0 + stage * C::kBBytes + crank * (C::kBBytes / kCtas);
          const int b_col = (kBMN && p.b_fold) ? (k0 / p.b_fold) * p.fold_cols : 0;
          const int b_row = (kBMN && p.b_fold) ? k0 % p.b_fold : k0;
          if (kAMN) {
#pragma unroll
            for (int j = 0; j < BM / 64; ++j) tc::tma_load_2d_u32(sa + j * 8192, &tmap_a, fb, m0 + 64 * j, k0);
          } else {
            tc::tma_load_2d_u32(sa, &tmap_a, fb, k0 + a_col, a_row);
          }
          if (kCtas == 2) {
            if (kBMN) {
#pragma unroll
              for (int j = 0; j < C::kBNCta / 64; ++j) tc::tma_load_2d_mc(sb + j * 8192, &tmap_b, fb, n0 + 64 * j + b_col, b_row, 3);
            } else {
              tc::tma_load_2d_mc(sb, &tmap_b, fb, k0, n0, 3);
            }
          } else {
            if (kBMN) {
#pragma unroll
              for (int j = 0; j < C::kBNCta / 64; ++j) tc::tma_load_2d_u32(sb + j * 8192, &tmap_b, fb, n0 + 64 * j + b_col, b_row);
            } else {
              tc::tma_load_2d_u32(sb, &tmap_b, fb, k0, n0);
            }
          }
        }
        __syncwarp();
        if (++stage == C::kStages) { stage = 0; phase ^= 1; }
      }
    }
  } else if (warp >= kConsWarp0) {
    const int wg = (warp - kConsWarp0) >> 2;
    const int wq = warp & 3;
    const uint32_t full0 = tc::smem_u32(full), empty0 = tc::smem_u32(empty);
    const uint32_t empty0_peer = kCtas == 2 ? mapa2(empty0, crank ^ 1u) : 0u;
    const uint64_t da0 = kAMN ? tc::desc_mnmajor_sw128(tc::smem_u32(smem_a) + wg * 8192) : tc::desc_kmajor_sw128(tc::smem_u32(smem_a) + wg * 8192);
    const uint64_t db0 = kBMN ? tc::desc_mnmajor_sw128(tc::smem_u32(smem_b)) : tc::desc_kmajor_sw128(tc::smem_u32(smem_b));
    constexpr uint64_t kAStep = kAMN ? (2048 >> 4) : (32 >> 4);
    constexpr uint64_t kBStep = kBMN ? (2048 >> 4) : (32 >> 4);
    auto release = [&](uint32_t st) {
      if (lane == 0) {
        tc::mbar_arrive_u32(empty0 + 8 * st);
        if (kCtas == 2) mbar_arrive_cluster(empty0_peer + 8 * st);
      }
    };
    uint32_t stage = 0, phase = 0;
    const int N = p.N, M = p.M;
    if (p.rowsum != nullptr) {
      reinterpret_cast<uint32_t*>(smem_ones)[threadIdx.x - kConsWarp0 * 32] = 0x3F803F80u;
      tc::fence_proxy_async();
      asm volatile("bar.sync 1, 256;" ::: "memory");
    }
    const uint64_t dones = tc::desc_kmajor_sw128(tc::smem_u32(smem_ones));
    for (int tile = cluster_id; tile < num_tiles; tile += num_clusters) {
      const int m0 = tile_m_of(tile) * TM + (int)crank * BM, n0 = (tile % tiles_n) * BN;
      const bool rs = p.rowsum != nullptr && n0 == 0;
      float acc[BN / 2];
      float rsum[4] = {0.f, 0.f, 0.f, 0.f};
#pragma unroll
      for (int i = 0; i < BN / 2; ++i) acc[i] = 0.f;
      uint32_t prev = 0;
      for (int kb = 0; kb < num_kb; ++kb) {
        while (!tc::mbar_try_wait_u32(full0 + 8 * stage, phase)) {}
        const uint64_t da = da0 + (uint64_t)(stage * (C::kABytes >> 4));
        const uint64_t db = db0 + (uint64_t)(stage * (C::kBBytes >> 4));
        tc::fence_regs(acc);
        tc::wgmma_fence();
#pragma unroll
        for (int k = 0; k < BK / 16; ++k)
          tc::Wgmma<BN, kAMN ? 1 : 0, kBMN ? 1 : 0>::mma(acc, da + k * kAStep, db + k * kBStep, (kb > 0 || k > 0) ? 1u : 0u);
        if (rs) {
          tc::fence_regs(rsum);
#pragma unroll
          for (int k = 0; k < BK / 16; ++k)
            tc::Wgmma<8, kAMN ? 1 : 0, 0>::mma(rsum, da + k * kAStep, dones + k * (32 >> 4), (kb > 0 || k > 0) ? 1u : 0u);
        }
        tc::wgmma_commit();
        tc::fence_regs(acc);
        tc::fence_regs(rsum);
        if (kb > 0) { tc::wgmma_wait<1>(); release(prev); }
        prev = stage;
        if (++stage == C::kStages) { stage = 0; phase ^= 1; }
      }
      tc::wgmma_wait<0>();
      tc::fence_regs(acc);
      tc::fence_regs(rsum);
      release(prev);
      if (rs && (lane & 3) == 0) {
#pragma unroll
        for (int h = 0; h < 2; ++h) {
          const int row = m0 + 64 * wg + tc::acc_row(2 * h, wq, lane);
          if (row < M) p.rowsum[row] = rsum[2 * h] + (p.rowsum_acc ? p.rowsum[row] : 0.f);
        }
      }
#pragma unroll
      for (int i = 0; i < BN / 2; i += 2) {
        const int row = m0 + 64 * wg + tc::acc_row(i, wq, lane);
        const int col = n0 + tc::acc_col(i, lane);
        if (row < M && col < N) {
          float f0 = acc[i], f1 = acc[i + 1];
          if (p.bias != nullptr) { f0 += p.bias[col]; f1 += p.bias[col + 1]; }
          if (kOut != OUT_BF16) {
            float2* dst = reinterpret_cast<float2*>(reinterpret_cast<float*>(p.C) + (size_t)row * p.ldc + col);
            if (kOut == OUT_F32_ACC) { const float2 o = *dst; f0 += o.x; f1 += o.y; }
            *dst = make_float2(f0, f1);
          } else {
            *reinterpret_cast<__nv_bfloat162*>(reinterpret_cast<__nv_bfloat16*>(p.C) + (size_t)row * p.ldc + col) =
                __floats2bfloat162_rn(f0, f1);
          }
        }
      }
      if (p.done != nullptr) {
        asm volatile("bar.sync 1, 256;" ::: "memory");
        if (warp == kConsWarp0 && lane == 0)
          asm volatile("red.release.gpu.global.add.u32 [%0], 1;"
                       ::"l"(p.done + ((size_t)tile_m_of(tile) * kCtas + crank) * tiles_n + (tile % tiles_n)) : "memory");
      }
    }
  }

  __syncthreads();
  if (kCtas == 2) cluster_sync2();
  if (p.pdl) asm volatile("griddepcontrol.wait;" ::: "memory");
}

template <int kCtas, int BN, bool kAMN, bool kBMN, int kOut>
int launch2(const void* A, const void* B, const Gemm2Params& p, int lda, int ldb, int dev, int max_ctas, cudaStream_t st) {
  using C = Cfg2<kCtas, BN>;
  CUtensorMap ta, tb;
  if (kAMN) { if (int rc = ts::make_tmap_2d_bf16(&ta, A, (uint64_t)p.K, (uint64_t)p.M, (uint64_t)lda, 64, BK)) return rc; }
  else if (p.a_fold) { if (int rc = ts::make_tmap_2d_bf16(&ta, A, (uint64_t)p.a_fold, (uint64_t)(p.M / p.a_fold) * p.fold_cols, (uint64_t)lda, BK, BM)) return rc; }
  else      { if (int rc = ts::make_tmap_2d_bf16(&ta, A, (uint64_t)p.M, (uint64_t)p.K, (uint64_t)lda, BK, BM)) return rc; }
  if (kBMN && p.b_fold) { if (int rc = ts::make_tmap_2d_bf16(&tb, B, (uint64_t)p.b_fold, (uint64_t)(p.K / p.b_fold) * p.fold_cols, (uint64_t)ldb, 64, BK)) return rc; }
  else if (kBMN) { if (int rc = ts::make_tmap_2d_bf16(&tb, B, (uint64_t)p.K, (uint64_t)p.N, (uint64_t)ldb, 64, BK)) return rc; }
  else      { if (int rc = ts::make_tmap_2d_bf16(&tb, B, (uint64_t)p.N, (uint64_t)p.K, (uint64_t)ldb, BK, C::kBNCta)) return rc; }
  auto kern = gemm2_kernel<kCtas, BN, kAMN, kBMN, kOut>;
  static bool attr_set = false;
  if (!attr_set) {
    cudaError_t e = cudaFuncSetAttribute(kern, cudaFuncAttributeMaxDynamicSharedMemorySize, C::kSmemBytes);
    if (e != cudaSuccess) return (int)e;
    cudaFuncSetAttribute(kern, cudaFuncAttributePreferredSharedMemoryCarveout, cudaSharedmemCarveoutMaxShared);
    attr_set = true;
  }
  const int TM = BM * kCtas;
  const int tiles = ((p.M + TM - 1) / TM) * ((p.N + BN - 1) / BN);
  int sms = ts::sm_count(dev);
  if (max_ctas > 0 && max_ctas < sms) sms = max_ctas;
  int clusters = sms / kCtas;
  if (clusters < 1) clusters = 1;
  if (tiles < clusters) clusters = tiles;
  cudaLaunchConfig_t cfg{};
  cfg.gridDim = dim3(clusters * kCtas); cfg.blockDim = dim3(kThreads); cfg.dynamicSmemBytes = C::kSmemBytes; cfg.stream = st;
  cudaLaunchAttribute at[2];
  at[0].id = cudaLaunchAttributeClusterDimension;
  at[0].val.clusterDim.x = kCtas; at[0].val.clusterDim.y = 1; at[0].val.clusterDim.z = 1;
  cfg.attrs = at; cfg.numAttrs = 1;
  if (p.pdl) {
    at[1].id = cudaLaunchAttributeProgrammaticStreamSerialization;
    at[1].val.programmaticStreamSerializationAllowed = 1;
    cfg.numAttrs = 2;
  }
  return (int)cudaLaunchKernelEx(&cfg, kern, ta, tb, p);
}

template <int kCtas, int BN, bool kAMN, bool kBMN>
int launch_out(const void* A, const void* B, const Gemm2Params& p, int lda, int ldb, int out_mode, int dev, int max_ctas, cudaStream_t st) {
  switch (out_mode) {
    case OUT_BF16: return launch2<kCtas, BN, kAMN, kBMN, OUT_BF16>(A, B, p, lda, ldb, dev, max_ctas, st);
    case OUT_F32: return launch2<kCtas, BN, kAMN, kBMN, OUT_F32>(A, B, p, lda, ldb, dev, max_ctas, st);
    case OUT_F32_ACC: return launch2<kCtas, BN, kAMN, kBMN, OUT_F32_ACC>(A, B, p, lda, ldb, dev, max_ctas, st);
  }
  return -3;
}

template <int kCtas, int BN>
int launch_major(const void* A, const void* B, const Gemm2Params& p, int lda, int ldb, int a_mn, int b_mn, int out_mode, int dev,
                 int max_ctas, cudaStream_t st) {
  if (a_mn && b_mn) return launch_out<kCtas, BN, true, true>(A, B, p, lda, ldb, out_mode, dev, max_ctas, st);
  if (a_mn) return launch_out<kCtas, BN, true, false>(A, B, p, lda, ldb, out_mode, dev, max_ctas, st);
  if (b_mn) return launch_out<kCtas, BN, false, true>(A, B, p, lda, ldb, out_mode, dev, max_ctas, st);
  return launch_out<kCtas, BN, false, false>(A, B, p, lda, ldb, out_mode, dev, max_ctas, st);
}

}

extern "C" int ts_gemm2(const void* A, const void* B, void* C, const float* bias, int M, int N, int K, int lda, int ldb, int ldc,
                        int a_mn, int b_mn, int out_mode, int ctas, int bn, int dev, int max_ctas, const unsigned int* gate,
                        const int* gate_cfg, unsigned int* done, int* gate_err, int pdl, int a_fold, int b_fold, int fold_cols,
                        float* rowsum, int rowsum_acc, cudaStream_t st) {
  if (M < 1 || N < 1 || K < 1) { ts::set_last_error("gemm2: M, N and K must be positive"); return -2; }
  if (K % 8 != 0 || lda % 8 != 0 || ldb % 8 != 0) { ts::set_last_error("gemm2: K and the operand pitches must be multiples of 8"); return -2; }
  if ((a_mn && M % 8 != 0) || (b_mn && N % 8 != 0) || N % 8 != 0) { ts::set_last_error("gemm2: M (MN-major A) / N must be multiples of 8"); return -2; }
  if (out_mode != OUT_BF16 && ldc % 2 != 0) { ts::set_last_error("gemm2: fp32 output needs an even row pitch"); return -2; }
  if (a_fold && (a_mn || gate != nullptr || a_fold % 128 != 0 || M % a_fold != 0 || K % 64 != 0 || fold_cols < K)) {
    ts::set_last_error("gemm2: folded A needs a K-major ungated operand, fold % 128 == 0, M % fold == 0, K % 64 == 0"); return -2;
  }
  if (b_fold && (!b_mn || b_fold % 64 != 0 || K % b_fold != 0 || N % bn != 0 || fold_cols < N)) {
    ts::set_last_error("gemm2: folded B needs an MN-major operand, fold % 64 == 0, K % fold == 0, N % bn == 0"); return -2;
  }
  if (rowsum != nullptr && out_mode == OUT_BF16) { ts::set_last_error("gemm2: row sums of A need an fp32 output"); return -2; }
  Gemm2Params p{};
  p.rowsum = rowsum; p.rowsum_acc = rowsum_acc;
  p.C = C; p.bias = bias; p.M = M; p.N = N; p.K = K; p.ldc = ldc;
  p.a_fold = a_fold; p.b_fold = b_fold; p.fold_cols = fold_cols;
  p.gate = gate; p.gate_err = gate_err; p.done = done; p.pdl = pdl;
  if (gate != nullptr) {
    p.gate_count = gate_cfg[0]; p.gate_stride = gate_cfg[1]; p.gate_base = gate_cfg[2]; p.gate_per_step = gate_cfg[3];
    p.gate_rows_per_step = gate_cfg[4] > 0 ? gate_cfg[4] : 1; p.gate_use_last = gate_cfg[5]; p.reverse_m = gate_cfg[6];
  }
  p.gate_spin_limit = 6000000000LL;
  if (ctas == 2) {
    if (bn == 128) return launch_major<2, 128>(A, B, p, lda, ldb, a_mn, b_mn, out_mode, dev, max_ctas, st);
    return launch_major<2, 256>(A, B, p, lda, ldb, a_mn, b_mn, out_mode, dev, max_ctas, st);
  }
  if (bn == 128) return launch_major<1, 128>(A, B, p, lda, ldb, a_mn, b_mn, out_mode, dev, max_ctas, st);
  return launch_major<1, 256>(A, B, p, lda, ldb, a_mn, b_mn, out_mode, dev, max_ctas, st);
}
```

### lstm_tensorspark_b200/ops/cuda_gemm.py

```python
from __future__ import annotations

import os
from typing import Optional

import torch

from .cuda_ext import ext

GEMM_CTAS = int(os.environ.get("LSTM_TS_GEMM_CTAS", "2"))
GEMM_BN = int(os.environ.get("LSTM_TS_GEMM_BN", "256"))
STATS = {"tc": 0, "generic": 0}


def _major(t: torch.Tensor):
    if t.dim() != 2:
        return None
    if t.stride(1) == 1 and t.stride(0) >= t.shape[1]:
        return False, t
    if t.stride(0) == 1 and t.stride(1) >= t.shape[0]:
        return True, t.t()
    return None


def _tc_ok(a_k: torch.Tensor, b_k: torch.Tensor, M: int, N: int, K: int) -> bool:
    if a_k.dtype != torch.bfloat16 or b_k.dtype != torch.bfloat16:
        return False
    if M < 128 or N < 16 or K < 64 or K % 8 or N % 8 or M % 8:
        return False
    for t in (a_k, b_k):
        if t.stride(0) % 8 or t.data_ptr() % 16:
            return False
    return True


def folded_ok(x_bm: torch.Tensor) -> bool:
    return (x_bm.is_cuda and x_bm.dim() == 3 and x_bm.dtype == torch.bfloat16 and x_bm.is_contiguous() and x_bm.shape[0] % 128 == 0
            and x_bm.shape[2] % max(64, GEMM_BN) == 0 and x_bm.data_ptr() % 16 == 0 and GEMM_BN in (128, 256))


def matmul(a: Optional[torch.Tensor], b_t: Optional[torch.Tensor], out: Optional[torch.Tensor] = None, accumulate: bool = False,
           out_dtype: Optional[torch.dtype] = None, bias: Optional[torch.Tensor] = None, max_ctas: int = 0,
           a_folded: Optional[torch.Tensor] = None, b_folded: Optional[torch.Tensor] = None, pdl: bool = False,
           ctas: int = 0, rowsum: Optional[tuple] = None) -> torch.Tensor:
    E = ext()
    ctas = ctas or GEMM_CTAS
    rs = dict(rowsum=rowsum[0], rowsum_acc=rowsum[1]) if rowsum is not None else {}
    if a_folded is not None or b_folded is not None:
        assert rowsum is None or a_folded is None, "row sums of a folded A are not supported"
        xb = a_folded if a_folded is not None else b_folded
        Bsz, T, F = xb.shape
        store = xb.view(Bsz, T * F)
        other = _major(b_t if a_folded is not None else a)
        assert folded_ok(xb) and other is not None and other[1].dtype == torch.bfloat16 and (a_folded is None or b_folded is None)
        if out_dtype is None:
            out_dtype = out.dtype if out is not None else torch.bfloat16
        STATS["tc"] += 1
        if a_folded is not None:
            return E.gemm2(store, other[1], bias=bias, out=out, a_mn=False, b_mn=other[0], out_fp32=out_dtype == torch.float32,
                           accumulate=accumulate, ctas=ctas, bn=GEMM_BN if b_t.shape[0] > 128 else 128, max_ctas=max_ctas, pdl=pdl,
                           a_fold=Bsz, fold_cols=F)
        return E.gemm2(other[1], store, bias=bias, out=out, a_mn=other[0], b_mn=True, out_fp32=out_dtype == torch.float32,
                       accumulate=accumulate, ctas=ctas, bn=GEMM_BN, max_ctas=max_ctas, pdl=pdl, b_fold=Bsz, fold_cols=F, **rs)
    M, K = a.shape
    N = b_t.shape[0]
    assert b_t.shape[1] == K, (a.shape, b_t.shape)
    if out_dtype is None:
        out_dtype = out.dtype if out is not None else a.dtype
    ma, mb = _major(a), _major(b_t)
    if ma is not None and mb is not None and _tc_ok(ma[1], mb[1], M, N, K) and out_dtype in (torch.bfloat16, torch.float32) \
            and not (accumulate and out_dtype != torch.float32) \
            and (out is None or (out.stride(1) == 1 and out.stride(0) % 4 == 0 and out.data_ptr() % 16 == 0)):
        STATS["tc"] += 1
        return E.gemm2(ma[1], mb[1], bias=bias, out=out, a_mn=ma[0], b_mn=mb[0], out_fp32=out_dtype == torch.float32,
                       accumulate=accumulate, ctas=ctas, bn=GEMM_BN if N > 128 else 128, max_ctas=max_ctas, pdl=pdl, **rs)
    assert a_folded is None and b_folded is None, "folded operands need the tensor-core path (check folded_ok first)"
    assert rowsum is None, "row sums need the tensor-core path"
    STATS["generic"] += 1
    a_g = a if a.dtype in (torch.float32, torch.bfloat16) else a.float()
    b_g = b_t if b_t.dtype in (torch.float32, torch.bfloat16) else b_t.float()
    if out is None:
        res = E.gemm_generic(a_g, b_g.t(), bias=bias, out_fp32=out_dtype == torch.float32)
        return res if res.dtype == out_dtype else res.to(out_dtype)
    return E.gemm_generic(a_g, b_g.t(), bias=bias, out=out, beta=1.0 if accumulate else 0.0)
```

### lstm_tensorspark_b200/ops/cuda_lstm.py

```python
from __future__ import annotations

import os
from typing import Optional

import torch

from .cuda_ext import ext
from . import cuda_gemm as G

_SYNC_WS = {}
_SM_COUNT = {}
FORCE_GENERIC = os.environ.get("LSTM_TS_FORCE_GENERIC", "0") == "1"
SEQ_VARIANT = int(os.environ.get("LSTM_TS_SEQ_VARIANT", "0"))
STATS = {"fast_fwd": 0, "fast_bwd": 0, "generic_fwd": 0, "generic_bwd": 0, "tc_gemm": 0, "kernels": 0}


HOOKS = {"grads_written": None}
AFTER_SEQ_BWD = []
_GEN = {"n": 0}


def queue_after_big_launch(fn):
    AFTER_SEQ_BWD.append((_GEN["n"], fn))


def _big_launch_begin():
    _GEN["n"] += 1


def _after_big_launch(flush: bool = False):
    while AFTER_SEQ_BWD and (flush or AFTER_SEQ_BWD[0][0] < _GEN["n"]):
        AFTER_SEQ_BWD.pop(0)[1]()


def _grads_written():
    h = HOOKS["grads_written"]
    if h is not None and not _CHUNKING["on"]:
        h()

_PARAMS = {}
DIRECT_GRADS = os.environ.get("LSTM_TS_DIRECT_GRADS", "1") == "1"


def register_param(addr: int, shadow: torch.Tensor, grad: torch.Tensor, owner=None) -> None:
    import weakref
    _PARAMS[addr] = (shadow, grad, weakref.ref(owner) if owner is not None else None)


def _lookup(addr: int):
    ent = _PARAMS.get(addr)
    if ent is None:
        return None
    if ent[2] is not None and ent[2]() is None:
        del _PARAMS[addr]
        return None
    return ent


def _lowp(w: torch.Tensor, cd: torch.dtype) -> torch.Tensor:
    if cd == torch.bfloat16:
        ent = _lookup(w.data_ptr())
        if ent is not None and ent[0].shape == w.shape:
            return ent[0]
    return w.detach().to(cd).contiguous()


def grad_sink(w_addr: int):
    ent = _lookup(w_addr) if DIRECT_GRADS else None
    if ent is None:
        return None
    owner = ent[2]() if ent[2] is not None else None
    if owner is None or w_addr not in owner._direct:
        if owner is not None:
            owner.ensure_zeroed(w_addr)
        return ent[1], True
    return ent[1], owner.take_sink(w_addr)


def _accumulate_grad(w_addr: int, a_t: torch.Tensor, b: torch.Tensor, b_folded: bool = False, pdl: bool = False,
                     max_ctas: int = 0, ctas: int = 0, rowsum=None):
    ops = dict(a=a_t, b_t=None, b_folded=b, ctas=ctas) if b_folded else dict(a=a_t, b_t=b.t(), ctas=ctas)
    ops["rowsum"] = rowsum
    if pdl:
        ops.update(pdl=True, ctas=1, max_ctas=max_ctas)
    sink = grad_sink(w_addr)
    if sink is not None:
        if not pdl:
            _big_launch_begin()
        G.matmul(out=sink[0], accumulate=sink[1], **ops)
        if not pdl:
            _after_big_launch()
        _grads_written()
        return None
    return G.matmul(out_dtype=torch.float32, **ops)


_BIAS_SPLIT = {}


def _bias_grad(b_addr: int, dg2d: torch.Tensor, under_gemm: bool = False, part: int = -1, max_ctas: int = 0):
    fast = dg2d.is_cuda and dg2d.dtype == torch.bfloat16 and dg2d.shape[1] % 512 == 0 and dg2d.is_contiguous()
    if part == 0:
        if not fast:
            return None
        sink = grad_sink(b_addr)
        _BIAS_SPLIT[b_addr] = sink
        if sink is None:
            return None
        half = dg2d.shape[1] // 2
        STATS["kernels"] += 1
        ext().colsum_bf16_into(dg2d, sink[0], not sink[1], under_gemm, 0, half)
        return None
    if part == 1 and fast and b_addr in _BIAS_SPLIT:
        sink = _BIAS_SPLIT.pop(b_addr)
        if sink is not None:
            half = dg2d.shape[1] // 2
            STATS["kernels"] += 1
            ext().colsum_bf16_into(dg2d, sink[0], not sink[1], under_gemm, half, half)
            _grads_written()
            return None
        return ext().colsum_bf16(dg2d)
    fast = dg2d.is_cuda and dg2d.dtype == torch.bfloat16 and dg2d.shape[1] % 256 == 0 and dg2d.is_contiguous()
    sink = grad_sink(b_addr)
    if fast:
        STATS["kernels"] += 1
        if sink is not None:
            ext().colsum_bf16_into(dg2d, sink[0], not sink[1], under_gemm and part < 0, max_ctas=max_ctas)
            _grads_written()
            return None
        return ext().colsum_bf16(dg2d)
    ones = torch.ones(1, dg2d.shape[0], dtype=dg2d.dtype, device=dg2d.device)
    if sink is not None:
        G.matmul(ones, dg2d.t(), out=sink[0].view(1, -1), accumulate=sink[1])
        _grads_written()
        return None
    return G.matmul(ones, dg2d.t(), out_dtype=torch.float32).view(-1)


SYNC_WORDS = 8192


def _sync_ws(device) -> torch.Tensor:
    key = (device.type, device.index)
    if key not in _SYNC_WS:
        _SYNC_WS[key] = torch.zeros(SYNC_WORDS, dtype=torch.int32, device=device)
    return _SYNC_WS[key]


def check_kernel_errors(device) -> None:
    ws = _SYNC_WS.get((device.type, device.index))
    if ws is not None and int(ws[SYNC_WORDS - 1].item()) != 0:
        raise RuntimeError("lstm_seq kernel aborted: an in-kernel wait timed out (see csrc/lstm_seq_wgmma.cu)")
    for (di, _tag), ent in list(globals().get("_WS_PAIR", {}).items()):
        if di == device.index and (int(ent[SYNC_WORDS - 1].item()) != 0 or int(ent[2 * SYNC_WORDS - 1].item()) != 0):
            raise RuntimeError("lstm_seq kernel (layer wavefront) aborted: an in-kernel wait timed out")


def _sms(device) -> int:
    key = device.index
    if key not in _SM_COUNT:
        _SM_COUNT[key] = torch.cuda.get_device_properties(device).multi_processor_count
    return _SM_COUNT[key]


_CORES = {}


def _coresident_ctas(device, cluster: int = 4) -> int:
    key = (device.index, cluster)
    if key not in _CORES:
        n = _sms(device)
        try:
            with torch.cuda.device(device):
                c = int(ext().lstm_seq_cluster_probe(cluster))
            if c > 0:
                n = min(n, cluster * c)
        except Exception:
            pass
        _CORES[key] = n
    return _CORES[key]


def _bwd_cluster(H: int) -> int:
    return 4 if H <= 1024 else 2


def _tiles_per_cta(B: int, H: int, device) -> Optional[int]:
    if H > 2048:
        return None
    tiles_m = (B + 127) // 128
    n = _coresident_ctas(device, _bwd_cluster(H))
    if tiles_m * (H // 16) <= n:
        return 1
    if H <= 1024 and tiles_m % 2 == 0 and (tiles_m // 2) * (H // 16) <= n:
        return 2
    return None


def _seq_variant(B: int, H: int, device) -> int:
    if SEQ_VARIANT & 15 or _tiles_per_cta(B, H, device) != 2:
        return SEQ_VARIANT
    return SEQ_VARIANT | 2


def fast_path_supported(B: int, H: int, dtype: torch.dtype, device) -> bool:
    if FORCE_GENERIC or dtype != torch.bfloat16 or H % 64 != 0:
        return False
    return (B + 127) // 128 <= 16 and _tiles_per_cta(B, H, device) is not None


def _batch_chunk(B: int, H: int, dtype: torch.dtype, device) -> Optional[int]:
    if FORCE_GENERIC or dtype != torch.bfloat16 or H % 64 != 0 or fast_path_supported(B, H, dtype, device):
        return None
    if H > 2048:
        return None
    tiles = _coresident_ctas(device, _bwd_cluster(H)) // (H // 16) * (2 if H <= 1024 else 1)
    if tiles < 1:
        return None
    chunk = min(tiles, 16) * 128
    return chunk if chunk < B else None


def _mm_f32(a: torch.Tensor, b: torch.Tensor) -> torch.Tensor:
    return G.matmul(a, b.t(), out_dtype=torch.float32)


def _transposed(w: torch.Tensor) -> torch.Tensor:
    if w.is_cuda and w.dim() == 2 and w.element_size() == 2 and w.is_contiguous():
        STATS["kernels"] += 1
        return ext().transpose2d(w)
    return w.t().contiguous()


def _gemm_tn(a: torch.Tensor, w: torch.Tensor) -> torch.Tensor:
    STATS["tc_gemm"] += 1
    STATS["kernels"] += 1
    return G.matmul(a, w, out_dtype=a.dtype)


_CHUNKING = {"on": False}


def _check_lengths_arg(lengths: Optional[torch.Tensor], B: int, device) -> None:
    if lengths is not None and (lengths.dtype != torch.int32 or lengths.shape != (B,) or lengths.device != device
                                or not lengths.is_contiguous()):
        raise ValueError(f"lengths must be a contiguous int32 [{B}] tensor on {device}, got {lengths.dtype} "
                         f"{tuple(lengths.shape)} on {lengths.device}")


def _drop_args(spec, device) -> dict:
    if spec is None or spec.p == 0:
        return {}
    step = spec.step
    if not isinstance(step, torch.Tensor):
        step = torch.tensor([int(step)], dtype=torch.int32, device=device)
    return {"drop_step": step, "drop_desc": spec.desc()}


class _DropoutFn(torch.autograd.Function):
    @staticmethod
    def forward(ctx, x, spec, t0):
        ctx.spec, ctx.t0 = spec, t0
        STATS["kernels"] += 1
        d = _drop_args(spec, x.device)
        return ext().dropout(x.contiguous(), d["drop_step"], d["drop_desc"], t0)

    @staticmethod
    def backward(ctx, g):
        STATS["kernels"] += 1
        d = _drop_args(ctx.spec, g.device)
        return ext().dropout(g.contiguous(), d["drop_step"], d["drop_desc"], ctx.t0), None, None


def dropout(x: torch.Tensor, spec, t0: int = 0) -> torch.Tensor:
    if spec is None or spec.p == 0:
        return x
    return _DropoutFn.apply(x, spec, t0)


class _LSTMSeqFn(torch.autograd.Function):
    @staticmethod
    def forward(ctx, x_seq, h0, c0, w_x, w_h, bias, lengths=None, reverse=False, dropout=None):
        E = ext()
        T, B, D = x_seq.shape
        H = w_h.shape[1]
        cd = x_seq.dtype
        x2d = x_seq.reshape(T * B, D).contiguous()
        w_x_c = _lowp(w_x, cd)
        w_h_c = _lowp(w_h, cd)
        bias_f = bias.detach().float().contiguous()
        gx = _gemm_tn(x2d, w_x_c).view(T, B, 4 * H)
        fast = fast_path_supported(B, H, cd, x_seq.device)
        c0f = c0.detach().float().contiguous()
        h0c = h0.detach().to(cd).contiguous()
        drop = _drop_args(dropout, x_seq.device)
        h_drop = None
        if fast:
            outs = E.lstm_seq_fwd(gx, w_h_c, bias_f, h0c, c0f, _sync_ws(x_seq.device), _seq_variant(B, H, x_seq.device),
                                  lengths=lengths, reverse=reverse, **drop)
            h_seq, c_seq, act = outs[:3]
            if drop:
                h_drop = outs[3]
            STATS["fast_fwd"] += 1
            STATS["kernels"] += 1
        else:
            h_seq = torch.empty(T + 1, B, H, dtype=cd, device=x_seq.device)
            c_seq = torch.empty(T + 1, B, H, dtype=torch.float32, device=x_seq.device)
            act = torch.empty(T, B, 4 * H, dtype=cd, device=x_seq.device)
            s0 = T if reverse else 0
            h_seq[s0].copy_(h0c)
            c_seq[s0].copy_(c0f)
            pre = torch.empty(B, 4 * H, dtype=cd, device=x_seq.device)
            for t in (range(T - 1, -1, -1) if reverse else range(T)):
                sp, sn = (t + 1, t) if reverse else (t, t + 1)
                pre.copy_(gx[t])
                G.matmul(h_seq[sp], w_h_c, out=pre, accumulate=True)
                h, c, a = E.lstm_pointwise_fwd(pre, bias_f, c_seq[sp], h_seq[sp], lengths, t)
                h_seq[sn].copy_(h)
                c_seq[sn].copy_(c)
                act[t].copy_(a)
            STATS["generic_fwd"] += 1
            STATS["kernels"] += T
            if drop:
                h_drop = E.dropout(h_seq[:T] if reverse else h_seq[1:], drop["drop_step"], drop["drop_desc"], 0)
                STATS["kernels"] += 1
        ctx.drop = drop
        ctx.save_for_backward(x2d, h_seq, c_seq, act, w_x_c, w_h_c)
        ctx.set_materialize_grads(False)
        ctx.fast = fast
        ctx.lengths = lengths
        ctx.reverse = reverse
        ctx.whole_batch = not _CHUNKING["on"]
        ctx.dims = (T, B, D, H)
        ctx.w_addrs = (w_x.data_ptr(), w_h.data_ptr(), bias.data_ptr())
        ctx.in_dtypes = (h0.dtype, c0.dtype)
        if reverse:
            return (h_seq[:T] if h_drop is None else h_drop), h_seq[0], c_seq[0]
        return (h_seq[1:] if h_drop is None else h_drop), h_seq[T], c_seq[T]

    @staticmethod
    def backward(ctx, dh_seq, dh_T, dc_T):
        E = ext()
        x2d, h_seq, c_seq, act, w_x_c, w_h_c = ctx.saved_tensors
        T, B, D, H = ctx.dims
        cd = act.dtype
        dev = act.device
        drop = ctx.drop if dh_seq is not None else {}
        if dh_seq is not None:
            dh_seq = dh_seq.to(cd).contiguous()
            if drop and not ctx.fast:
                dh_seq = E.dropout(dh_seq, drop["drop_step"], drop["drop_desc"], 0)
                STATS["kernels"] += 1
        elif not ctx.fast:
            dh_seq = torch.zeros(T, B, H, dtype=cd, device=dev)
        dcT = (dc_T.float().contiguous() if dc_T is not None else torch.zeros(B, H, dtype=torch.float32, device=dev))
        dhT = (dh_T.float().contiguous() if dh_T is not None else torch.zeros(B, H, dtype=torch.float32, device=dev))
        if ctx.fast:
            w_hT = _transposed(w_h_c)
            _big_launch_begin()
            dpre, dh0, dc0 = E.lstm_seq_bwd(dh_seq, w_hT, act, c_seq, dhT, dcT, _sync_ws(dev), _seq_variant(B, H, dev),
                                            lengths=ctx.lengths, reverse=ctx.reverse, **drop)
            STATS["fast_bwd"] += 1
            STATS["kernels"] += 1
            _after_big_launch()
        else:
            dpre = torch.empty_like(act)
            dh_rec: Optional[torch.Tensor] = dhT if dh_T is not None else None
            dc = dcT
            for t in (range(T) if ctx.reverse else range(T - 1, -1, -1)):
                sp, sn = (t + 1, t) if ctx.reverse else (t, t + 1)
                if ctx.lengths is None:
                    dp, dc = E.lstm_pointwise_bwd(dh_seq[t], dh_rec, dc, act[t], c_seq[sp], c_seq[sn])
                    dh_rec = _mm_f32(dp, w_h_c)
                else:
                    dp, dc, dh_pass = E.lstm_pointwise_bwd(dh_seq[t], dh_rec, dc, act[t], c_seq[sp], c_seq[sn], ctx.lengths, t)
                    G.matmul(dp, w_h_c.t(), out=dh_pass, accumulate=True)
                    dh_rec = dh_pass
                dpre[t].copy_(dp)
            dh0, dc0 = dh_rec, dc
            STATS["generic_bwd"] += 1
            STATS["kernels"] += T
        dg2d = dpre.view(T * B, 4 * H)
        dg_t = dg2d.t()
        dw_x = _accumulate_grad(ctx.w_addrs[0], dg_t, x2d)
        h_prev = h_seq[1:] if ctx.reverse else h_seq[:T]
        dw_h = _accumulate_grad(ctx.w_addrs[1], dg_t, h_prev.reshape(T * B, H))
        db = _bias_grad(ctx.w_addrs[2], dg2d)
        dx = None
        if ctx.needs_input_grad[0]:
            dx = G.matmul(dg2d, w_x_c.t(), out_dtype=cd).view(T, B, D)
            STATS["kernels"] += 1
        h0_dt, c0_dt = ctx.in_dtypes
        return dx, dh0.to(h0_dt), dc0.to(c0_dt), dw_x, dw_h, db, None, None, None


def lstm_layer_sequence(x_seq, h0, c0, w_x, w_h, bias, lengths=None, reverse=False, dropout=None):
    if (not x_seq.is_contiguous() and not x_seq.requires_grad and x_seq.transpose(0, 1).is_contiguous()
            and (x_seq.shape[2] * x_seq.element_size()) % 16 == 0):
        x_seq = ext().transpose01(x_seq.transpose(0, 1))
        STATS["kernels"] += 1
    T, B, _ = x_seq.shape
    H = w_h.shape[1]
    _check_lengths_arg(lengths, B, x_seq.device)
    chunk = _batch_chunk(B, H, x_seq.dtype, x_seq.device)
    if chunk is not None:
        _CHUNKING["on"] = True
        try:
            outs = [_LSTMSeqFn.apply(x_seq[:, b0:b0 + chunk].contiguous(), h0[b0:b0 + chunk], c0[b0:b0 + chunk], w_x, w_h, bias,
                                     None if lengths is None else lengths[b0:b0 + chunk], reverse,
                                     None if dropout is None else dropout.at_rows(b0))
                    for b0 in range(0, B, chunk)]
        finally:
            _CHUNKING["on"] = False
        STATS["batch_chunks"] = STATS.get("batch_chunks", 0) + len(outs)
        return (torch.cat([o[0] for o in outs], dim=1), torch.cat([o[1] for o in outs], dim=0),
                torch.cat([o[2] for o in outs], dim=0))
    return _LSTMSeqFn.apply(x_seq.contiguous(), h0, c0, w_x, w_h, bias, lengths, reverse, dropout)


FOLDED_FEED = os.environ.get("LSTM_TS_FOLDED_FEED", "1") != "0"
WAVEFRONT = os.environ.get("LSTM_TS_WAVEFRONT", "1") == "1"
_SIDE_STREAMS = {}
_WS_PAIR = {}


def _side_streams(device):
    key = device.index
    if key not in _SIDE_STREAMS:
        _SIDE_STREAMS[key] = (torch.cuda.Stream(device=device), torch.cuda.Stream(device=device))
    return _SIDE_STREAMS[key]


_WARM = set()


def _warm_wavefront_kernels(device):
    if device.index in _WARM:
        return
    a = torch.zeros(256, 64, dtype=torch.bfloat16, device=device)
    w = torch.zeros(256, 64, dtype=torch.bfloat16, device=device)
    wt = torch.zeros(64, 256, dtype=torch.bfloat16, device=device)
    ext().gemm2(a, w, ctas=1, bn=256)
    ext().gemm2(a, wt, b_mn=True, ctas=1, bn=256)
    torch.cuda.synchronize(device)
    _WARM.add(device.index)


def _pair_ws(device, tag: str, n_done: int):
    key = (device.index, tag)
    ent = _WS_PAIR.get(key)
    if ent is None or ent.numel() < 2 * SYNC_WORDS + n_done:
        ent = torch.zeros(2 * SYNC_WORDS + max(n_done, 1), dtype=torch.int32, device=device)
        _WS_PAIR[key] = ent
    return ent[:SYNC_WORDS], ent[SYNC_WORDS:2 * SYNC_WORDS], ent[2 * SYNC_WORDS:2 * SYNC_WORDS + n_done]


def pair_schedule(T: int, B: int, D: int, h_a: int, h_b: int, sms: int, coresident: int) -> Optional[str]:
    if B != 256 or T < 2 or D % 8 != 0 or any(h % 256 != 0 or h > 1024 for h in (h_a, h_b)):
        return None
    both = h_a // 16 + h_b // 16 + 8
    if both <= coresident + 16 and both <= sms:
        return "wavefront"
    if max(h_a, h_b) // 16 <= coresident and max(h_a, h_b) // 16 + 8 <= sms:
        return "pipelined"
    return None


def pipelined_fwd_split(sms: int, d: int, h_a: int, h_b: int) -> tuple:
    free = max(2, sms - h_a // 16)
    n_a = min(free - 1, max(1, round(free * d / (d + h_b)))) if d > 0 else 0
    return n_a, free - n_a


def _pair_schedule_of(x_seq: torch.Tensor, h_a: int, h_b: int) -> Optional[str]:
    if not (WAVEFRONT and x_seq.is_cuda and x_seq.dtype == torch.bfloat16 and not FORCE_GENERIC and x_seq.dim() == 3):
        return None
    if (SEQ_VARIANT & 15) > 2:
        return None
    T, B, D = x_seq.shape
    return pair_schedule(T, B, D, h_a, h_b, _sms(x_seq.device), _coresident_ctas(x_seq.device))


def wavefront_supported(x_seq: torch.Tensor, h_a: int, h_b: int) -> bool:
    return _pair_schedule_of(x_seq, h_a, h_b) is not None


WAVE_SYNC_MODE = int(os.environ.get("LSTM_TS_WAVE_SYNC", "1"))


def _wave_variant() -> int:
    return (SEQ_VARIANT & ~(15 | (3 << 16))) | 2 | ((WAVE_SYNC_MODE & 1) << 16)


_COLSUM_SMS = 4


def _pair_variant(schedule: str) -> int:
    var = _wave_variant()
    return var & ~(3 << 16) if schedule == "pipelined" else var


def _gate_off(var: int) -> int:
    return 0 if (var >> 16) & 3 == 1 else 512


def _gate_cfg(var: int, tiles_m: int, nkb: int, per_kb_step: int, ctas_per_tile: int, base_steps: int, step_sign: int, rows: int, bwd: bool):
    if (var >> 16) & 3 == 1:
        per = ctas_per_tile
        return [tiles_m, 1, per * base_steps, per * step_sign, rows, 0 if bwd else 1, 1 if bwd else 0]
    per = per_kb_step
    return [tiles_m * nkb, 32, per * base_steps, per * step_sign, rows, 0 if bwd else 1, 1 if bwd else 0]


class _LSTMPairFn(torch.autograd.Function):
    @staticmethod
    def forward(ctx, x_seq, h0a, c0a, w_xa, w_ha, b_a, h0b, c0b, w_xb, w_hb, b_b, lengths=None, schedule="wavefront", drop_a=None,
                drop_b=None):
        E = ext()
        pipelined = schedule == "pipelined"
        dev = x_seq.device
        T, B, D = x_seq.shape
        Ha, Hb = w_ha.shape[1], w_hb.shape[1]
        cd = x_seq.dtype
        x_bm = x_seq.transpose(0, 1) if not x_seq.is_contiguous() else None
        x2d = x_seq.reshape(T * B, D) if x_bm is None else x_bm
        wxa, wha, wxb, whb = _lowp(w_xa, cd), _lowp(w_ha, cd), _lowp(w_xb, cd), _lowp(w_hb, cd)
        ba_f, bb_f = b_a.detach().float().contiguous(), b_b.detach().float().contiguous()
        h0a_c, h0b_c = h0a.detach().to(cd).contiguous(), h0b.detach().to(cd).contiguous()
        c0a_f, c0b_f = c0a.detach().float().contiguous(), c0b.detach().float().contiguous()
        _warm_wavefront_kernels(dev)
        opt = dict(dtype=cd, device=dev)
        side_a = pipelined and D >= 64
        if side_a:
            gx_a = torch.empty(T, B, 4 * Ha, **opt)
        elif x_bm is None:
            gx_a = _gemm_tn(x2d, wxa).view(T, B, 4 * Ha)
        else:
            STATS["tc_gemm"] += 1; STATS["kernels"] += 1; STATS["folded_feed"] = STATS.get("folded_feed", 0) + 1
            gx_a = G.matmul(None, wxa, out_dtype=cd, a_folded=x_bm).view(T, B, 4 * Ha)
        h_seq_a = torch.empty(T + 1, B, Ha, **opt); c_seq_a = torch.empty(T + 1, B, Ha, dtype=torch.float32, device=dev)
        act_a = torch.empty(T, B, 4 * Ha, **opt); til_a = torch.empty((T + 1) * 2 * 128 * Ha, **opt)
        h_seq_b = torch.empty(T + 1, B, Hb, **opt); c_seq_b = torch.empty(T + 1, B, Hb, dtype=torch.float32, device=dev)
        act_b = torch.empty(T, B, 4 * Hb, **opt); til_b = torch.empty((T + 1) * 2 * 128 * Hb, **opt)
        gx_b = torch.empty(T, B, 4 * Hb, **opt)
        dra, drb = _drop_args(drop_a, dev), _drop_args(drop_b, dev)
        h_drop_a = torch.empty(T, B, Ha, **opt) if dra else None
        h_drop_b = torch.empty(T, B, Hb, **opt) if drb else None
        hin_b = h_seq_a[1:] if h_drop_a is None else h_drop_a
        tn, tn_a = 4 * Hb // 256, 4 * Ha // 256
        ws_a, ws_b, done = _pair_ws(dev, "fwd", T * 2 * (tn + (tn_a if side_a else 0)))
        done.zero_()
        done, done_a = done[:T * 2 * tn], done[T * 2 * tn:]
        var = _pair_variant(schedule)
        E.lstm_seq_prologue(h0a_c, c0a_f, h_seq_a, c_seq_a, til_a, ws_a)
        E.lstm_seq_prologue(h0b_c, c0b_f, h_seq_b, c_seq_b, til_b, ws_b)
        E.lstm_seq_fwd_into(gx_a, wha, ba_f, h0a_c, c0a_f, h_seq_a, c_seq_a, act_a, til_a, ws_a, var, done_a if side_a else None,
                            tn_a if side_a else 0, True, 0, 1, lengths, h_drop=h_drop_a, **dra)
        if pipelined:
            ctas_a, free_ctas = pipelined_fwd_split(_sms(dev), D if side_a else 0, Ha, Hb)
        if side_a:
            a_op = dict(A=x2d, a_fold=0) if x_bm is None else dict(A=x_bm.reshape(B, T * D), a_fold=B, fold_cols=D)
            E.gemm2(B=wxa, out=gx_a.view(T * B, 4 * Ha), ctas=1, bn=256, max_ctas=ctas_a, done=done_a, pdl=True, **a_op)
            STATS["tc_gemm"] += 1; STATS["kernels"] += 1; STATS["pipelined_side_gemms"] = STATS.get("pipelined_side_gemms", 0) + 1
            if x_bm is not None:
                STATS["folded_feed"] = STATS.get("folded_feed", 0) + 1
        if not pipelined:
            E.lstm_seq_fwd_into(gx_b, whb, bb_f, h0b_c, c0b_f, h_seq_b, c_seq_b, act_b, til_b, ws_b, var, done, tn, False, 0, 3, lengths,
                                h_drop=h_drop_b, **drb)
            free_ctas = max(1, _sms(dev) - Ha // 16 - Hb // 16)
        E.gemm2(hin_b.view(T * B, Ha), wxb, out=gx_b.view(T * B, 4 * Hb), ctas=1, bn=256, max_ctas=free_ctas,
                gate=ws_a[_gate_off(var):], gate_cfg=_gate_cfg(var, 2, Ha // 64, 4, 4 * Ha // 64, 2, 1, B, False), done=done,
                gate_err=ws_a[SYNC_WORDS - 1:], pdl=True)
        if pipelined:
            E.lstm_seq_fwd_into(gx_b, whb, bb_f, h0b_c, c0b_f, h_seq_b, c_seq_b, act_b, til_b, ws_b, var, None, 0, False, 0, 1, lengths,
                                h_drop=h_drop_b, **drb)
        STATS["fast_fwd"] += 2
        STATS["kernels"] += 3
        STATS[schedule + "_fwd"] = STATS.get(schedule + "_fwd", 0) + 1
        ctx.save_for_backward(x2d, h_seq_a, c_seq_a, act_a, h_seq_b, c_seq_b, act_b, wxa, wha, wxb, whb, hin_b)
        ctx.set_materialize_grads(False)
        ctx.drop = (dra, drb)
        ctx.dims = (T, B, D, Ha, Hb)
        ctx.lengths = lengths
        ctx.pipelined = pipelined
        ctx.x_folded = x_bm is not None
        ctx.addrs = (w_xa.data_ptr(), w_ha.data_ptr(), b_a.data_ptr(), w_xb.data_ptr(), w_hb.data_ptr(), b_b.data_ptr())
        ctx.in_dtypes = (h0a.dtype, c0a.dtype, h0b.dtype, c0b.dtype)
        return (h_seq_b[1:] if h_drop_b is None else h_drop_b), h_seq_a[T], c_seq_a[T], h_seq_b[T], c_seq_b[T]

    @staticmethod
    def backward(ctx, dh_seq_b, dhT_a, dcT_a, dhT_b, dcT_b):
        E = ext()
        x2d, h_seq_a, c_seq_a, act_a, h_seq_b, c_seq_b, act_b, wxa, wha, wxb, whb, hin_b = ctx.saved_tensors
        dra, drb = ctx.drop
        if dh_seq_b is None:
            drb = {}
        T, B, D, Ha, Hb = ctx.dims
        cd, dev = act_a.dtype, act_a.device
        if dh_seq_b is not None:
            dh_seq_b = dh_seq_b.to(cd).contiguous()
        f32 = dict(dtype=torch.float32, device=dev)
        z = lambda g, H: g.float().contiguous().clone() if g is not None else torch.zeros(B, H, **f32)
        dh0a, dc0a, dh0b, dc0b = z(dhT_a, Ha), z(dcT_a, Ha), z(dhT_b, Hb), z(dcT_b, Hb)
        whT_a, whT_b = _transposed(wha), _transposed(whb)
        dpre_a = torch.empty_like(act_a); dpre_b = torch.empty_like(act_b)
        til_a = torch.empty(T * 2 * 128 * 4 * Ha, dtype=cd, device=dev); til_b = torch.empty(T * 2 * 128 * 4 * Hb, dtype=cd, device=dev)
        dx_b = torch.empty(T, B, Ha, dtype=cd, device=dev)
        tn = Ha // 256
        ws_b, ws_a, done = _pair_ws(dev, "bwd", T * tn * 2)
        ws_a[:SYNC_WORDS - 1].zero_(); ws_b[:SYNC_WORDS - 1].zero_(); done.zero_()
        var = _pair_variant("pipelined" if ctx.pipelined else "wavefront")
        pipelined = ctx.pipelined
        E.lstm_seq_bwd_into(dh_seq_b, whT_b, act_b, c_seq_b, dpre_b, dh0b, dc0b, til_b, ws_b, var, None, 0, True, 0, 1, ctx.lengths, **drb)
        if not pipelined:
            E.lstm_seq_bwd_into(dx_b, whT_a, act_a, c_seq_a, dpre_a, dh0a, dc0a, til_a, ws_a, var, done, tn, False, 0, 3, ctx.lengths,
                                **dra)
        free_ctas = max(1, _sms(dev) - Hb // 16 - (0 if pipelined else Ha // 16))
        E.gemm2(dpre_b.view(T * B, 4 * Hb), wxb, out=dx_b.view(T * B, Ha), b_mn=True, ctas=1, bn=256, max_ctas=free_ctas,
                gate=ws_b[_gate_off(var):], gate_cfg=_gate_cfg(var, 2, 4 * Hb // 64, 1, 4 * Hb // 64, T + 1, -1, B, True), done=done,
                gate_err=ws_b[SYNC_WORDS - 1:], pdl=True)
        if pipelined:
            E.lstm_seq_bwd_into(dx_b, whT_a, act_a, c_seq_a, dpre_a, dh0a, dc0a, til_a, ws_a, var, None, 0, False, 0, 1, ctx.lengths, **dra)
        STATS["fast_bwd"] += 2
        STATS["kernels"] += 5
        a = ctx.addrs
        dg_b = dpre_b.view(T * B, 4 * Hb)
        if pipelined:
            side = max(1, (_sms(dev) - Ha // 16 - _COLSUM_SMS) // 2)
            dw_xb = _accumulate_grad(a[3], dg_b.t(), hin_b.reshape(T * B, Ha), pdl=True, max_ctas=side)
            dw_hb = _accumulate_grad(a[4], dg_b.t(), h_seq_b[:T].reshape(T * B, Hb), pdl=True, max_ctas=side)
            db_b = _bias_grad(a[5], dg_b, under_gemm=True, max_ctas=4 * _COLSUM_SMS)
        else:
            dw_xb = _accumulate_grad(a[3], dg_b.t(), hin_b.reshape(T * B, Ha))
            _bias_grad(a[5], dg_b, under_gemm=dw_xb is None, part=0)
            dw_hb = _accumulate_grad(a[4], dg_b.t(), h_seq_b[:T].reshape(T * B, Hb))
            db_b = _bias_grad(a[5], dg_b, under_gemm=dw_hb is None, part=1)
        dg_a = dpre_a.view(T * B, 4 * Ha)
        if pipelined:
            dw_xa = _accumulate_grad(a[0], dg_a.t(), x2d, b_folded=ctx.x_folded, ctas=1)
            bsink = grad_sink(a[2])
            db_a = bsink[0] if bsink is not None else torch.empty(4 * Ha, **f32)
            dw_ha = _accumulate_grad(a[1], dg_a.t(), h_seq_a[:T].reshape(T * B, Ha), ctas=1,
                                     rowsum=(db_a, bsink is not None and bsink[1]))
            STATS["fused_bias_grads"] = STATS.get("fused_bias_grads", 0) + 1
            if bsink is not None:
                db_a = None
                _grads_written()
        else:
            dw_xa = _accumulate_grad(a[0], dg_a.t(), x2d, b_folded=ctx.x_folded)
            _bias_grad(a[2], dg_a, under_gemm=dw_xa is None, part=0)
            dw_ha = _accumulate_grad(a[1], dg_a.t(), h_seq_a[:T].reshape(T * B, Ha))
            db_a = _bias_grad(a[2], dg_a, under_gemm=dw_ha is None, part=1)
        dx = None
        if ctx.needs_input_grad[0]:
            dx = G.matmul(dg_a, wxa.t(), out_dtype=cd).view(T, B, D)
            STATS["kernels"] += 1
        t = ctx.in_dtypes
        return (dx, dh0a.to(t[0]), dc0a.to(t[1]), dw_xa, dw_ha, db_a, dh0b.to(t[2]), dc0b.to(t[3]), dw_xb, dw_hb, db_b, None, None,
                None, None)


def lstm_pair_sequence(x_seq, la, lb, lengths=None, schedule=None, dropouts=(None, None)):
    _check_lengths_arg(lengths, x_seq.shape[1], x_seq.device)
    if schedule is None:
        schedule = _pair_schedule_of(x_seq, la[3].shape[1], lb[3].shape[1])
    if schedule not in ("wavefront", "pipelined"):
        raise ValueError(f"no layer-pair schedule for x {tuple(x_seq.shape)} {x_seq.dtype}, H = {la[3].shape[1]}, "
                         f"{lb[3].shape[1]} (schedule={schedule!r}); check wavefront_supported first")
    if (not x_seq.is_contiguous() and not x_seq.requires_grad and x_seq.transpose(0, 1).is_contiguous()
            and (x_seq.shape[2] * x_seq.element_size()) % 16 == 0):
        if FOLDED_FEED and G.folded_ok(x_seq.transpose(0, 1)):
            return _LSTMPairFn.apply(x_seq, *la, *lb, lengths, schedule, *dropouts)
        x_seq = ext().transpose01(x_seq.transpose(0, 1))
        STATS["kernels"] += 1
    return _LSTMPairFn.apply(x_seq.contiguous(), *la, *lb, lengths, schedule, *dropouts)
```

Baseline: 22340.

## Chunk weight-gradient GEMMs and gate them to overlap the LSTM backward recurrence

Adds a chunked wgrad GEMM mode that walks the time dimension backwards in chunks. Before each chunk it waits on the recurrent backward kernel's progress counters, so dW and db accumulation can start while the backward recurrence is still running. The mode fuses two B operands and the bias row-sum into one launch, and splits SMs between the dx GEMM and the wgrad work using a rate model. The cost is extra fp32 read-modify-write of the gradient outputs for every chunk, plus spin-waiting CTAs that compete with the recurrence.

Result: faster. 22570 (median of 6 runs) (+1.0%).

```diff
diff --git a/lstm_tensorspark_b200/csrc/bindings.cpp b/lstm_tensorspark_b200/csrc/bindings.cpp
--- a/lstm_tensorspark_b200/csrc/bindings.cpp
+++ b/lstm_tensorspark_b200/csrc/bindings.cpp
@@ -63,6 +63,8 @@
                     int, int, int, float, cudaStream_t);
 int ts_gemm2(const void*, const void*, void*, const float*, int, int, int, int, int, int, int, int, int, int, int, int, int,
              const unsigned int*, const int*, unsigned int*, int*, int, int, int, int, float*, int, cudaStream_t);
+int ts_gemm2_wgrad(const void*, const void*, const void*, void*, void*, int, int, int, int, int, int, int, int, int, int, int, int,
+                   int, int, int, const unsigned int*, const int*, int*, int, int, int, float*, int, cudaStream_t);
 int ts_lstm_seq_fwd(const void*, const void*, const float*, const void*, const float*, void*, const float*, void*, void*, int,
                     int, int, unsigned int*, int, cudaStream_t, const void*, const unsigned int*, int, int, int, const int*, int,
                     void*, const int*, const unsigned int*);
@@ -751,6 +753,51 @@
                  gate_err.has_value() ? gate_err->data_ptr<int>() : nullptr, pdl ? 1 : 0, (int)a_fold, (int)b_fold, (int)fold_cols,
                  rp, rowsum_acc ? 1 : 0, stream_handle ? (cudaStream_t)stream_handle : stream()), "gemm2");
   return C;
+}
+
+void gemm2_wgrad(const Tensor& A, const Tensor& B, const std::optional<Tensor>& B2, Tensor C, const std::optional<Tensor>& C2,
+                 bool accumulate, int64_t chunk_rows, int64_t k_begin, int64_t k_end, int64_t max_ctas, const std::optional<Tensor>& gate,
+                 const std::vector<int64_t>& gate_cfg, const std::optional<Tensor>& gate_err, bool pdl, int64_t b_fold, int64_t fold_cols,
+                 const std::optional<Tensor>& rowsum, bool rowsum_acc) {
+  auto bf = [](const Tensor& t) { return t.is_cuda() && t.scalar_type() == torch::kBFloat16 && t.dim() == 2 && t.stride(1) == 1; };
+  auto f32 = [](const Tensor& t) { return t.is_cuda() && t.scalar_type() == torch::kFloat32 && t.dim() == 2 && t.stride(1) == 1; };
+  TORCH_CHECK(bf(A) && bf(B) && (!B2.has_value() || bf(*B2)), "gemm2_wgrad: A, B, B2 must be 2-D bf16 CUDA tensors with unit inner stride");
+  TORCH_CHECK(f32(C) && (!C2.has_value() || f32(*C2)), "gemm2_wgrad: C, C2 must be 2-D fp32 CUDA tensors with unit inner stride");
+  TORCH_CHECK(B2.has_value() == C2.has_value(), "gemm2_wgrad: B2 and C2 go together");
+  c10::cuda::CUDAGuard gd(A.device());
+  const int K = A.size(0), M = A.size(1);
+  if (b_fold) {
+    TORCH_CHECK(B.size(0) == b_fold && fold_cols > 0 && B.size(1) % fold_cols == 0 && b_fold * (B.size(1) / fold_cols) == K,
+                "gemm2_wgrad: folded B must be [fold, T * fold_cols] with T * fold = K");
+  } else {
+    TORCH_CHECK(B.size(0) == K, "gemm2_wgrad: B must have K = ", K, " rows");
+  }
+  const int N = b_fold ? (int)fold_cols : (int)B.size(1);
+  TORCH_CHECK(C.size(0) == M && C.size(1) == N, "gemm2_wgrad: C must be [M, N]");
+  int N2 = 0;
+  if (B2.has_value()) {
+    N2 = B2->size(1);
+    TORCH_CHECK(B2->size(0) == K && C2->size(0) == M && C2->size(1) == N2, "gemm2_wgrad: B2 must be [K, N2] and C2 [M, N2]");
+  }
+  const unsigned int* gp = nullptr;
+  int gcfg[7] = {0, 0, 0, 0, 1, 0, 0};
+  if (gate.has_value()) {
+    TORCH_CHECK(gate->is_cuda() && gate->scalar_type() == torch::kInt32 && gate_cfg.size() == 7, "gemm2_wgrad: gate int32 cuda + 7 config ints");
+    gp = (const unsigned int*)gate->data_ptr<int>();
+    for (int i = 0; i < 7; ++i) gcfg[i] = (int)gate_cfg[i];
+  }
+  float* rp = nullptr;
+  if (rowsum.has_value()) {
+    TORCH_CHECK(rowsum->is_cuda() && rowsum->scalar_type() == torch::kFloat32 && rowsum->is_contiguous() && rowsum->numel() == M,
+                "gemm2_wgrad: rowsum must be a contiguous fp32 [M]");
+    rp = rowsum->data_ptr<float>();
+  }
+  check(ts_gemm2_wgrad(A.data_ptr(), B.data_ptr(), B2.has_value() ? B2->data_ptr() : nullptr, C.data_ptr(),
+                       C2.has_value() ? C2->data_ptr() : nullptr, M, N, N2, K, (int)A.stride(0), (int)B.stride(0),
+                       B2.has_value() ? (int)B2->stride(0) : 0, (int)C.stride(0), C2.has_value() ? (int)C2->stride(0) : 0,
+                       accumulate ? 1 : 0, (int)chunk_rows, (int)k_begin, (int)k_end, A.device().index(), (int)max_ctas, gp, gcfg,
+                       gate_err.has_value() ? gate_err->data_ptr<int>() : nullptr, pdl ? 1 : 0, (int)b_fold, (int)fold_cols, rp,
+                       rowsum_acc ? 1 : 0, stream()), "gemm2_wgrad");
 }
 
 Tensor gemm_generic(const Tensor& A, const Tensor& B, const std::optional<Tensor>& bias, std::optional<Tensor> out, bool out_fp32, double beta) {
@@ -960,6 +1007,10 @@
         py::arg("max_ctas") = 0, py::arg("gate") = py::none(), py::arg("gate_cfg") = std::vector<int64_t>{}, py::arg("done") = py::none(),
         py::arg("gate_err") = py::none(), py::arg("stream") = 0, py::arg("pdl") = false, py::arg("a_fold") = 0, py::arg("b_fold") = 0,
         py::arg("fold_cols") = 0, py::arg("rowsum") = py::none(), py::arg("rowsum_acc") = false);
+  m.def("gemm2_wgrad", &gemm2_wgrad, py::arg("A"), py::arg("B"), py::arg("B2") = py::none(), py::arg("C"), py::arg("C2") = py::none(),
+        py::arg("accumulate") = false, py::arg("chunk_rows"), py::arg("k_begin"), py::arg("k_end"), py::arg("max_ctas") = 0,
+        py::arg("gate") = py::none(), py::arg("gate_cfg") = std::vector<int64_t>{}, py::arg("gate_err") = py::none(), py::arg("pdl") = false,
+        py::arg("b_fold") = 0, py::arg("fold_cols") = 0, py::arg("rowsum") = py::none(), py::arg("rowsum_acc") = false);
   m.def("lstm_seq_fwd", &lstm_seq_fwd, py::arg("gx"), py::arg("w_h"), py::arg("bias"), py::arg("h0"), py::arg("c0"),
         py::arg("sync_ws"), py::arg("variant") = 0, py::arg("dbg") = py::none(), py::arg("in_gate") = py::none(),
         py::arg("in_gate_tiles_n") = 0, py::arg("extra_signal") = false, py::arg("lengths") = py::none(), py::arg("reverse") = false,
diff --git a/lstm_tensorspark_b200/csrc/gemm2_wgmma.cu b/lstm_tensorspark_b200/csrc/gemm2_wgmma.cu
--- a/lstm_tensorspark_b200/csrc/gemm2_wgmma.cu
+++ b/lstm_tensorspark_b200/csrc/gemm2_wgmma.cu
@@ -54,11 +54,35 @@
   int a_fold, b_fold, fold_cols;
   float* rowsum;
   int rowsum_acc;
+  void* C2;
+  int N2, ldc2;
+  int chunk_rows, k_begin, k_end, acc_first;
 };
 
-template <int kCtas, int BN, bool kAMN, bool kBMN, int kOut>
+TC_DEVICE bool gate_wait(const Gemm2Params& p, int t, int lane) {
+  const int target = p.gate_base + p.gate_per_step * t;
+  const long long t0 = clock64();
+  bool ok = true;
+  for (int g = lane; g < p.gate_count; g += 32) {
+    const unsigned int* c = p.gate + (size_t)g * p.gate_stride;
+    unsigned int v;
+    while (true) {
+      asm volatile("ld.relaxed.gpu.global.u32 %0, [%1];" : "=r"(v) : "l"(c) : "memory");
+      if ((int)v - target >= 0) break;
+      if (clock64() - t0 > p.gate_spin_limit) { if (p.gate_err) atomicExch(p.gate_err, 1); ok = false; break; }
+    }
+  }
+  ok = __all_sync(0xffffffffu, ok);
+  asm volatile("fence.acq_rel.gpu;" ::: "memory");
+  asm volatile("fence.proxy.async.global;" ::: "memory");
+  return ok;
+}
+
+template <int kCtas, int BN, bool kAMN, bool kBMN, int kOut, bool kChunk = false>
 __global__ void __launch_bounds__(kThreads, 1)
-gemm2_kernel(const __grid_constant__ CUtensorMap tmap_a, const __grid_constant__ CUtensorMap tmap_b, const Gemm2Params p) {
+gemm2_kernel(const __grid_constant__ CUtensorMap tmap_a, const __grid_constant__ CUtensorMap tmap_b,
+             const __grid_constant__ CUtensorMap tmap_b2, const Gemm2Params p) {
+  static_assert(!kChunk || (kCtas == 1 && kAMN && kBMN && kOut == OUT_F32_ACC), "chunked mode: dW = dG^T · X, single-CTA tiles");
   using C = Cfg2<kCtas, BN>;
   extern __shared__ uint8_t smem_raw[];
   uint8_t* smem = reinterpret_cast<uint8_t*>((reinterpret_cast<uintptr_t>(smem_raw) + 1023) & ~uintptr_t(1023));
@@ -84,6 +108,7 @@
   if (warp == 0 && lane == 0) {
     tc::prefetch_tmap(&tmap_a);
     tc::prefetch_tmap(&tmap_b);
+    if (kChunk && p.C2 != nullptr) tc::prefetch_tmap(&tmap_b2);
   }
   if (warp == 1 && lane == 0) {
     for (int s = 0; s < C::kStages; ++s) { tc::mbar_init(&full[s], 1); tc::mbar_init(&empty[s], 8 * kCtas); }
@@ -92,35 +117,55 @@
   __syncthreads();
   if (kCtas == 2) cluster_sync2();
 
-  if (warp == 0) {
+  const int tn0 = kChunk ? tiles_n : 0, tn1 = (kChunk && p.C2 != nullptr) ? (p.N2 + BN - 1) / BN : 0;
+  const int chunk_tiles = tiles_m * (tn0 + tn1);
+
+  if (kChunk && warp == 0) {
     const uint32_t full0 = tc::smem_u32(full), empty0 = tc::smem_u32(empty);
     const uint32_t sa0 = tc::smem_u32(smem_a), sb0 = tc::smem_u32(smem_b);
     uint32_t stage = 0, phase = 0;
-    bool ok = true;
+    bool gate_dead = false;
+    for (int kh = p.k_end; kh > p.k_begin; kh -= p.chunk_rows) {
+      const int kl = max(p.k_begin, kh - p.chunk_rows);
+      if (p.gate != nullptr && !gate_dead)
+        gate_dead = !gate_wait(p, kl / p.gate_rows_per_step, lane);
+      for (int tile = blockIdx.x; tile < chunk_tiles; tile += gridDim.x) {
+        const bool second = tile >= tiles_m * tn0;
+        const int local = second ? tile - tiles_m * tn0 : tile, tnp = second ? tn1 : tn0;
+        const int m0 = (local / tnp) * BM, n0 = (local % tnp) * BN;
+        const CUtensorMap* tb = second ? &tmap_b2 : &tmap_b;
+        const int fold = second ? 0 : p.b_fold;
+        for (int k0 = kl; k0 < kh; k0 += BK) {
+          const uint32_t eb = empty0 + 8 * stage, fb = full0 + 8 * stage;
+          while (!tc::mbar_try_wait_u32(eb, phase ^ 1)) {}
+          if (tc::elect_one()) {
+            tc::mbar_expect_tx_u32(fb, C::kStageBytes);
+            const uint32_t sa = sa0 + stage * C::kABytes, sb = sb0 + stage * C::kBBytes;
+            const int b_col = fold ? (k0 / fold) * p.fold_cols : 0, b_row = fold ? k0 % fold : k0;
+#pragma unroll
+            for (int j = 0; j < BM / 64; ++j) tc::tma_load_2d_u32(sa + j * 8192, &tmap_a, fb, m0 + 64 * j, k0);
+#pragma unroll
+            for (int j = 0; j < BN / 64; ++j) tc::tma_load_2d_u32(sb + j * 8192, tb, fb, n0 + 64 * j + b_col, b_row);
+          }
+          __syncwarp();
+          if (++stage == C::kStages) { stage = 0; phase ^= 1; }
+        }
+      }
+    }
+  } else if (!kChunk && warp == 0) {
+    const uint32_t full0 = tc::smem_u32(full), empty0 = tc::smem_u32(empty);
+    const uint32_t sa0 = tc::smem_u32(smem_a), sb0 = tc::smem_u32(smem_b);
+    uint32_t stage = 0, phase = 0;
     int gate_t_ok = -1;
     bool gate_dead = false;
-    for (int tile = cluster_id; tile < num_tiles && ok; tile += num_clusters) {
+    for (int tile = cluster_id; tile < num_tiles; tile += num_clusters) {
       const int m0 = tile_m_of(tile) * TM + (int)crank * BM;
       const int n0 = (tile % tiles_n) * BN + (int)crank * C::kBNCta;
       if (p.gate != nullptr) {
         const int r0 = tile_m_of(tile) * TM, r1 = min(r0 + TM, p.M) - 1;
         const int t = (p.gate_use_last ? r1 : r0) / p.gate_rows_per_step;
         if (t != gate_t_ok && !gate_dead) {
-          const int target = p.gate_base + p.gate_per_step * t;
-          const long long t0 = clock64();
-          for (int g = lane; g < p.gate_count; g += 32) {
-            const unsigned int* c = p.gate + (size_t)g * p.gate_stride;
-            unsigned int v;
-            while (true) {
-              asm volatile("ld.relaxed.gpu.global.u32 %0, [%1];" : "=r"(v) : "l"(c) : "memory");
-              if ((int)v - target >= 0) break;
-              if (clock64() - t0 > p.gate_spin_limit) { if (p.gate_err) atomicExch(p.gate_err, 1); ok = false; break; }
-            }
-          }
-          ok = __all_sync(0xffffffffu, ok);
-          asm volatile("fence.acq_rel.gpu;" ::: "memory");
-          asm volatile("fence.proxy.async.global;" ::: "memory");
-          if (!ok) { gate_dead = true; ok = true; }
+          if (!gate_wait(p, t, lane)) gate_dead = true;
           gate_t_ok = t;
         }
       }
@@ -184,6 +229,71 @@
       asm volatile("bar.sync 1, 256;" ::: "memory");
     }
     const uint64_t dones = tc::desc_kmajor_sw128(tc::smem_u32(smem_ones));
+    if constexpr (kChunk) {
+    for (int kh = p.k_end; kh > p.k_begin; kh -= p.chunk_rows) {
+      const int kb_n = (kh - max(p.k_begin, kh - p.chunk_rows)) / BK;
+      const bool old = kh != p.k_end || p.acc_first, rs_old = kh != p.k_end || p.rowsum_acc;
+      for (int tile = blockIdx.x; tile < chunk_tiles; tile += gridDim.x) {
+        const bool second = tile >= tiles_m * tn0;
+        const int local = second ? tile - tiles_m * tn0 : tile, tnp = second ? tn1 : tn0;
+        const int m0 = (local / tnp) * BM, n0 = (local % tnp) * BN;
+        const bool rs = p.rowsum != nullptr;
+        float acc[BN / 2];
+        float rsum[4] = {0.f, 0.f, 0.f, 0.f};
+#pragma unroll
+        for (int i = 0; i < BN / 2; ++i) acc[i] = 0.f;
+        uint32_t prev = 0;
+        for (int kb = 0; kb < kb_n; ++kb) {
+          while (!tc::mbar_try_wait_u32(full0 + 8 * stage, phase)) {}
+          const uint64_t da = da0 + (uint64_t)(stage * (C::kABytes >> 4));
+          const uint64_t db = db0 + (uint64_t)(stage * (C::kBBytes >> 4));
+          tc::fence_regs(acc);
+          tc::wgmma_fence();
+#pragma unroll
+          for (int k = 0; k < BK / 16; ++k) tc::Wgmma<BN, 1, 1>::mma(acc, da + k * kAStep, db + k * kBStep, (kb > 0 || k > 0) ? 1u : 0u);
+          if (rs) {
+            tc::fence_regs(rsum);
+#pragma unroll
+            for (int k = 0; k < BK / 16; ++k) tc::Wgmma<8, 1, 0>::mma(rsum, da + k * kAStep, dones + k * (32 >> 4), (kb > 0 || k > 0) ? 1u : 0u);
+          }
+          tc::wgmma_commit();
+          tc::fence_regs(acc);
+          tc::fence_regs(rsum);
+          if (kb > 0) { tc::wgmma_wait<1>(); release(prev); }
+          prev = stage;
+          if (++stage == C::kStages) { stage = 0; phase ^= 1; }
+        }
+        tc::wgmma_wait<0>();
+        tc::fence_regs(acc);
+        tc::fence_regs(rsum);
+        release(prev);
+        if (rs && n0 == 0 && !second && (lane & 3) == 0) {
+#pragma unroll
+          for (int h = 0; h < 2; ++h) {
+            const int row = m0 + 64 * wg + tc::acc_row(2 * h, wq, lane);
+            if (row < M) p.rowsum[row] = rsum[2 * h] + (rs_old ? p.rowsum[row] : 0.f);
+          }
+        }
+        float* const out = reinterpret_cast<float*>(second ? p.C2 : p.C);
+        const int ldc = second ? p.ldc2 : p.ldc, Np = second ? p.N2 : N;
+        if (old) {
+#pragma unroll
+          for (int i = 0; i < BN / 2; i += 2) {
+            const int row = m0 + 64 * wg + tc::acc_row(i, wq, lane), col = n0 + tc::acc_col(i, lane);
+            if (row < M && col < Np) {
+              const float2 o = *reinterpret_cast<const float2*>(out + (size_t)row * ldc + col);
+              acc[i] += o.x; acc[i + 1] += o.y;
+            }
+          }
+        }
+#pragma unroll
+        for (int i = 0; i < BN / 2; i += 2) {
+          const int row = m0 + 64 * wg + tc::acc_row(i, wq, lane), col = n0 + tc::acc_col(i, lane);
+          if (row < M && col < Np) *reinterpret_cast<float2*>(out + (size_t)row * ldc + col) = make_float2(acc[i], acc[i + 1]);
+        }
+      }
+    }
+    } else {
     for (int tile = cluster_id; tile < num_tiles; tile += num_clusters) {
       const int m0 = tile_m_of(tile) * TM + (int)crank * BM, n0 = (tile % tiles_n) * BN;
       const bool rs = p.rowsum != nullptr && n0 == 0;
@@ -249,6 +359,7 @@
                        ::"l"(p.done + ((size_t)tile_m_of(tile) * kCtas + crank) * tiles_n + (tile % tiles_n)) : "memory");
       }
     }
+    }
   }
 
   __syncthreads();
@@ -256,17 +367,20 @@
   if (p.pdl) asm volatile("griddepcontrol.wait;" ::: "memory");
 }
 
-template <int kCtas, int BN, bool kAMN, bool kBMN, int kOut>
-int launch2(const void* A, const void* B, const Gemm2Params& p, int lda, int ldb, int dev, int max_ctas, cudaStream_t st) {
+template <int kCtas, int BN, bool kAMN, bool kBMN, int kOut, bool kChunk = false>
+int launch2(const void* A, const void* B, const Gemm2Params& p, int lda, int ldb, int dev, int max_ctas, cudaStream_t st,
+            const void* B2 = nullptr, int ldb2 = 0) {
   using C = Cfg2<kCtas, BN>;
-  CUtensorMap ta, tb;
+  CUtensorMap ta, tb, tb2;
   if (kAMN) { if (int rc = ts::make_tmap_2d_bf16(&ta, A, (uint64_t)p.K, (uint64_t)p.M, (uint64_t)lda, 64, BK)) return rc; }
   else if (p.a_fold) { if (int rc = ts::make_tmap_2d_bf16(&ta, A, (uint64_t)p.a_fold, (uint64_t)(p.M / p.a_fold) * p.fold_cols, (uint64_t)lda, BK, BM)) return rc; }
   else      { if (int rc = ts::make_tmap_2d_bf16(&ta, A, (uint64_t)p.M, (uint64_t)p.K, (uint64_t)lda, BK, BM)) return rc; }
   if (kBMN && p.b_fold) { if (int rc = ts::make_tmap_2d_bf16(&tb, B, (uint64_t)p.b_fold, (uint64_t)(p.K / p.b_fold) * p.fold_cols, (uint64_t)ldb, 64, BK)) return rc; }
   else if (kBMN) { if (int rc = ts::make_tmap_2d_bf16(&tb, B, (uint64_t)p.K, (uint64_t)p.N, (uint64_t)ldb, 64, BK)) return rc; }
   else      { if (int rc = ts::make_tmap_2d_bf16(&tb, B, (uint64_t)p.N, (uint64_t)p.K, (uint64_t)ldb, BK, C::kBNCta)) return rc; }
-  auto kern = gemm2_kernel<kCtas, BN, kAMN, kBMN, kOut>;
+  if (B2 != nullptr) { if (int rc = ts::make_tmap_2d_bf16(&tb2, B2, (uint64_t)p.K, (uint64_t)p.N2, (uint64_t)ldb2, 64, BK)) return rc; }
+  else tb2 = tb;
+  auto kern = gemm2_kernel<kCtas, BN, kAMN, kBMN, kOut, kChunk>;
   static bool attr_set = false;
   if (!attr_set) {
     cudaError_t e = cudaFuncSetAttribute(kern, cudaFuncAttributeMaxDynamicSharedMemorySize, C::kSmemBytes);
@@ -275,7 +389,7 @@
     attr_set = true;
   }
   const int TM = BM * kCtas;
-  const int tiles = ((p.M + TM - 1) / TM) * ((p.N + BN - 1) / BN);
+  const int tiles = ((p.M + TM - 1) / TM) * ((p.N + BN - 1) / BN + (B2 != nullptr ? (p.N2 + BN - 1) / BN : 0));
   int sms = ts::sm_count(dev);
   if (max_ctas > 0 && max_ctas < sms) sms = max_ctas;
   int clusters = sms / kCtas;
@@ -292,7 +406,7 @@
     at[1].val.programmaticStreamSerializationAllowed = 1;
     cfg.numAttrs = 2;
   }
-  return (int)cudaLaunchKernelEx(&cfg, kern, ta, tb, p);
+  return (int)cudaLaunchKernelEx(&cfg, kern, ta, tb, tb2, p);
 }
 
 template <int kCtas, int BN, bool kAMN, bool kBMN>
@@ -348,3 +462,33 @@
   if (bn == 128) return launch_major<1, 128>(A, B, p, lda, ldb, a_mn, b_mn, out_mode, dev, max_ctas, st);
   return launch_major<1, 256>(A, B, p, lda, ldb, a_mn, b_mn, out_mode, dev, max_ctas, st);
 }
+
+extern "C" int ts_gemm2_wgrad(const void* A, const void* B, const void* B2, void* C, void* C2, int M, int N, int N2, int K, int lda,
+                              int ldb, int ldb2, int ldc, int ldc2, int acc_first, int chunk_rows, int k_begin, int k_end, int dev,
+                              int max_ctas, const unsigned int* gate, const int* gate_cfg, int* gate_err, int pdl, int b_fold,
+                              int fold_cols, float* rowsum, int rowsum_acc, cudaStream_t st) {
+  if (M < 1 || N < 1 || K < 1 || (B2 != nullptr && N2 < 1)) { ts::set_last_error("gemm2_wgrad: M, N, N2 and K must be positive"); return -2; }
+  if (M % 8 != 0 || N % 8 != 0 || (B2 != nullptr && N2 % 8 != 0) || lda % 8 != 0 || ldb % 8 != 0 || ldb2 % 8 != 0 ||
+      ldc % 2 != 0 || ldc2 % 2 != 0) {
+    ts::set_last_error("gemm2_wgrad: M, N, N2 and the operand pitches must be multiples of 8, the output pitches even"); return -2;
+  }
+  if (chunk_rows < BK || chunk_rows % BK != 0 || k_begin < 0 || k_begin % BK != 0 || k_end > K || k_end % BK != 0 || k_begin >= k_end) {
+    ts::set_last_error("gemm2_wgrad: chunk_rows, k_begin and k_end must be multiples of 64 with 0 <= k_begin < k_end <= K"); return -2;
+  }
+  if (b_fold && (b_fold % 64 != 0 || K % b_fold != 0 || N % 256 != 0 || fold_cols < N)) {
+    ts::set_last_error("gemm2_wgrad: folded B needs fold % 64 == 0, K % fold == 0, N % 256 == 0"); return -2;
+  }
+  Gemm2Params p{};
+  p.C = C; p.M = M; p.N = N; p.K = K; p.ldc = ldc;
+  p.C2 = B2 != nullptr ? C2 : nullptr; p.N2 = N2; p.ldc2 = ldc2;
+  p.chunk_rows = chunk_rows; p.k_begin = k_begin; p.k_end = k_end; p.acc_first = acc_first;
+  p.b_fold = b_fold; p.fold_cols = fold_cols;
+  p.rowsum = rowsum; p.rowsum_acc = rowsum_acc;
+  p.gate = gate; p.gate_err = gate_err; p.pdl = pdl;
+  if (gate != nullptr) {
+    p.gate_count = gate_cfg[0]; p.gate_stride = gate_cfg[1]; p.gate_base = gate_cfg[2]; p.gate_per_step = gate_cfg[3];
+    p.gate_rows_per_step = gate_cfg[4] > 0 ? gate_cfg[4] : 1;
+  }
+  p.gate_spin_limit = 6000000000LL;
+  return launch2<1, 256, true, true, OUT_F32_ACC, true>(A, B, p, lda, ldb, dev, max_ctas, st, B2, ldb2);
+}
diff --git a/lstm_tensorspark_b200/ops/cuda_gemm.py b/lstm_tensorspark_b200/ops/cuda_gemm.py
--- a/lstm_tensorspark_b200/ops/cuda_gemm.py
+++ b/lstm_tensorspark_b200/ops/cuda_gemm.py
@@ -82,3 +82,20 @@
         res = E.gemm_generic(a_g, b_g.t(), bias=bias, out_fp32=out_dtype == torch.float32)
         return res if res.dtype == out_dtype else res.to(out_dtype)
     return E.gemm_generic(a_g, b_g.t(), bias=bias, out=out, beta=1.0 if accumulate else 0.0)
+
+
+def wgrad_chunked(dg: torch.Tensor, bs: list, outs: list, accumulate: bool, chunk_rows: int, k_begin: int, k_end: int,
+                  max_ctas: int = 0, gate: Optional[torch.Tensor] = None, gate_cfg=(), gate_err: Optional[torch.Tensor] = None,
+                  pdl: bool = False, rowsum: Optional[tuple] = None, b_folded: bool = False) -> None:
+    assert 1 <= len(bs) == len(outs) <= 2
+    fold = {}
+    b0 = bs[0]
+    if b_folded:
+        Bsz, T, F = b0.shape
+        assert folded_ok(b0)
+        b0, fold = b0.view(Bsz, T * F), dict(b_fold=Bsz, fold_cols=F)
+    rs = dict(rowsum=rowsum[0], rowsum_acc=rowsum[1]) if rowsum is not None else {}
+    STATS["tc"] += 1
+    ext().gemm2_wgrad(dg, b0, bs[1] if len(bs) > 1 else None, outs[0], outs[1] if len(outs) > 1 else None, accumulate=accumulate,
+                      chunk_rows=chunk_rows, k_begin=k_begin, k_end=k_end, max_ctas=max_ctas, gate=gate, gate_cfg=list(gate_cfg),
+                      gate_err=gate_err, pdl=pdl, **fold, **rs)
diff --git a/lstm_tensorspark_b200/ops/cuda_lstm.py b/lstm_tensorspark_b200/ops/cuda_lstm.py
--- a/lstm_tensorspark_b200/ops/cuda_lstm.py
+++ b/lstm_tensorspark_b200/ops/cuda_lstm.py
@@ -98,7 +98,7 @@
 _BIAS_SPLIT = {}
 
 
-def _bias_grad(b_addr: int, dg2d: torch.Tensor, under_gemm: bool = False, part: int = -1, max_ctas: int = 0):
+def _bias_grad(b_addr: int, dg2d: torch.Tensor, under_gemm: bool = False, part: int = -1):
     fast = dg2d.is_cuda and dg2d.dtype == torch.bfloat16 and dg2d.shape[1] % 512 == 0 and dg2d.is_contiguous()
     if part == 0:
         if not fast:
@@ -125,7 +125,7 @@
     if fast:
         STATS["kernels"] += 1
         if sink is not None:
-            ext().colsum_bf16_into(dg2d, sink[0], not sink[1], under_gemm and part < 0, max_ctas=max_ctas)
+            ext().colsum_bf16_into(dg2d, sink[0], not sink[1], under_gemm and part < 0)
             _grads_written()
             return None
         return ext().colsum_bf16(dg2d)
@@ -442,6 +442,8 @@
     wt = torch.zeros(64, 256, dtype=torch.bfloat16, device=device)
     ext().gemm2(a, w, ctas=1, bn=256)
     ext().gemm2(a, wt, b_mn=True, ctas=1, bn=256)
+    c = torch.empty(256, 256, dtype=torch.float32, device=device)
+    ext().gemm2_wgrad(wt, wt, C=c, chunk_rows=64, k_begin=0, k_end=64)
     torch.cuda.synchronize(device)
     _WARM.add(device.index)
 
@@ -492,7 +494,53 @@
     return (SEQ_VARIANT & ~(15 | (3 << 16))) | 2 | ((WAVE_SYNC_MODE & 1) << 16)
 
 
-_COLSUM_SMS = 4
+WGRAD_CHUNK = 32
+WGRAD_TAIL = 32
+WGRAD_B_REST = 32
+_DX_RATE, _DW_RATE = 5.1, 6.75
+
+
+def chunk_plan(T: int, L: int, tail: int) -> list:
+    return [(max(tail, t1 - L), t1) for t1 in range(T, tail, -L)] + [(0, min(T, tail))]
+
+
+def pipelined_bwd_split(sms: int, h_a: int, h_b: int) -> tuple:
+    free = max(2, sms - h_b // 16)
+    dx, dw = h_a / _DX_RATE, (h_a + h_b) / _DW_RATE
+    n1 = min(free - 1, max(1, round(free * dx / (dx + dw))))
+    return n1, free - n1
+
+
+def pipelined_bwd_rest_split(sms: int, d: int, h_a: int, h_b: int, rows_b: int, rows_a: int) -> tuple:
+    free = max(2, sms - h_a // 16)
+    if rows_a <= 0:
+        return free, 0
+    wb, wa = rows_b * h_b * (h_a + h_b), rows_a * h_a * (d + h_a)
+    n_b = min(free - 1, max(1, round(free * wb / (wb + wa))))
+    return n_b, free - n_b
+
+
+def _wgrad_sinks(w_addrs, shapes, dev):
+    sinks, ret = [], []
+    for addr, shape in zip(w_addrs, shapes):
+        sink = grad_sink(addr)
+        sinks.append((sink[0], bool(sink[1])) if sink is not None else (torch.empty(*shape, dtype=torch.float32, device=dev), False))
+        ret.append(None if sink is not None else sinks[-1][0])
+    ws = sinks[:-1]
+    if len({acc for _, acc in ws}) > 1:
+        for out, acc in ws:
+            if not acc:
+                out.zero_()
+        sinks = [(out, True) for out, _ in ws] + sinks[-1:]
+    return sinks, ret
+
+
+def _chunked_wgrads(dg, bs, sinks, rows_per_step, k_begin, k_end, first, b_folded=False, **launch):
+    n = len(bs)
+    G.wgrad_chunked(dg, bs, [o for o, _ in sinks[:n]], sinks[0][1] or not first, WGRAD_CHUNK * rows_per_step, k_begin, k_end,
+                    rowsum=(sinks[-1][0], sinks[-1][1] or not first), b_folded=b_folded, **launch)
+    STATS["kernels"] += 1
+    STATS["chunked_wgrads"] = STATS.get("chunked_wgrads", 0) + 1
 
 
 def _pair_variant(schedule: str) -> int:
@@ -611,42 +659,52 @@
         ws_a[:SYNC_WORDS - 1].zero_(); ws_b[:SYNC_WORDS - 1].zero_(); done.zero_()
         var = _pair_variant("pipelined" if ctx.pipelined else "wavefront")
         pipelined = ctx.pipelined
+        a = ctx.addrs
+        dg_b, dg_a = dpre_b.view(T * B, 4 * Hb), dpre_a.view(T * B, 4 * Ha)
         E.lstm_seq_bwd_into(dh_seq_b, whT_b, act_b, c_seq_b, dpre_b, dh0b, dc0b, til_b, ws_b, var, None, 0, True, 0, 1, ctx.lengths, **drb)
         if not pipelined:
             E.lstm_seq_bwd_into(dx_b, whT_a, act_a, c_seq_a, dpre_a, dh0a, dc0a, til_a, ws_a, var, done, tn, False, 0, 3, ctx.lengths,
                                 **dra)
-        free_ctas = max(1, _sms(dev) - Hb // 16 - (0 if pipelined else Ha // 16))
-        E.gemm2(dpre_b.view(T * B, 4 * Hb), wxb, out=dx_b.view(T * B, Ha), b_mn=True, ctas=1, bn=256, max_ctas=free_ctas,
-                gate=ws_b[_gate_off(var):], gate_cfg=_gate_cfg(var, 2, 4 * Hb // 64, 1, 4 * Hb // 64, T + 1, -1, B, True), done=done,
-                gate_err=ws_b[SYNC_WORDS - 1:], pdl=True)
+        gcfg = lambda H: _gate_cfg(var, 2, 4 * H // 64, 1, 4 * H // 64, T + 1, -1, B, True)
         if pipelined:
+            n_dx, n_wb = pipelined_bwd_split(_sms(dev), Ha, Hb)
+        else:
+            n_dx = max(1, _sms(dev) - Hb // 16 - Ha // 16)
+        E.gemm2(dg_b, wxb, out=dx_b.view(T * B, Ha), b_mn=True, ctas=1, bn=256, max_ctas=n_dx, gate=ws_b[_gate_off(var):],
+                gate_cfg=gcfg(Hb), done=done, gate_err=ws_b[SYNC_WORDS - 1:], pdl=True)
+        if pipelined:
+            plan_b, plan_a = chunk_plan(T, WGRAD_CHUNK, WGRAD_B_REST), chunk_plan(T, WGRAD_CHUNK, WGRAD_TAIL)
+            kb_mid, ka_mid, k_end = plan_b[-1][1] * B, plan_a[-1][1] * B, T * B
+            side_xa = D >= 64
+            bs_b = [hin_b.reshape(T * B, Ha), h_seq_b[:T].reshape(T * B, Hb)]
+            bs_a = ([x2d] if side_xa else []) + [h_seq_a[:T].reshape(T * B, Ha)]
+            sinks_b, ret_b = _wgrad_sinks(a[3:6], [(4 * Hb, Ha), (4 * Hb, Hb), (4 * Hb,)], dev)
+            sinks_a, ret_a = _wgrad_sinks((a[0:3] if side_xa else a[1:3]), ([(4 * Ha, D)] if side_xa else []) + [(4 * Ha, Ha), (4 * Ha,)],
+                                          dev)
+            fold_a = ctx.x_folded and side_xa
+            if len(plan_b) > 1:
+                _chunked_wgrads(dg_b, bs_b, sinks_b, B, kb_mid, k_end, True, max_ctas=n_wb, gate=ws_b[_gate_off(var):],
+                                gate_cfg=gcfg(Hb), gate_err=ws_b[SYNC_WORDS - 1:], pdl=True)
             E.lstm_seq_bwd_into(dx_b, whT_a, act_a, c_seq_a, dpre_a, dh0a, dc0a, til_a, ws_a, var, None, 0, False, 0, 1, ctx.lengths, **dra)
+            n_rest, n_a = pipelined_bwd_rest_split(_sms(dev), D if side_xa else 0, Ha, Hb, kb_mid, k_end - ka_mid)
+            _chunked_wgrads(dg_b, bs_b, sinks_b, B, 0, kb_mid, len(plan_b) == 1, max_ctas=n_rest, pdl=True)
+            if len(plan_a) > 1:
+                _chunked_wgrads(dg_a, bs_a, sinks_a, B, ka_mid, k_end, True, b_folded=fold_a, max_ctas=n_a,
+                                gate=ws_a[_gate_off(var):], gate_cfg=gcfg(Ha), gate_err=ws_a[SYNC_WORDS - 1:], pdl=True)
+            _big_launch_begin()
+            _chunked_wgrads(dg_a, bs_a, sinks_a, B, 0, ka_mid, len(plan_a) == 1, b_folded=fold_a)
+            _after_big_launch()
+            dw_xb, dw_hb, db_b = ret_b
+            dw_xa = _accumulate_grad(a[0], dg_a.t(), x2d, b_folded=ctx.x_folded, ctas=1) if not side_xa else ret_a[0]
+            dw_ha, db_a = ret_a[-2:]
+            _grads_written()
         STATS["fast_bwd"] += 2
         STATS["kernels"] += 5
-        a = ctx.addrs
-        dg_b = dpre_b.view(T * B, 4 * Hb)
-        if pipelined:
-            side = max(1, (_sms(dev) - Ha // 16 - _COLSUM_SMS) // 2)
-            dw_xb = _accumulate_grad(a[3], dg_b.t(), hin_b.reshape(T * B, Ha), pdl=True, max_ctas=side)
-            dw_hb = _accumulate_grad(a[4], dg_b.t(), h_seq_b[:T].reshape(T * B, Hb), pdl=True, max_ctas=side)
-            db_b = _bias_grad(a[5], dg_b, under_gemm=True, max_ctas=4 * _COLSUM_SMS)
-        else:
+        if not pipelined:
             dw_xb = _accumulate_grad(a[3], dg_b.t(), hin_b.reshape(T * B, Ha))
             _bias_grad(a[5], dg_b, under_gemm=dw_xb is None, part=0)
             dw_hb = _accumulate_grad(a[4], dg_b.t(), h_seq_b[:T].reshape(T * B, Hb))
             db_b = _bias_grad(a[5], dg_b, under_gemm=dw_hb is None, part=1)
-        dg_a = dpre_a.view(T * B, 4 * Ha)
-        if pipelined:
-            dw_xa = _accumulate_grad(a[0], dg_a.t(), x2d, b_folded=ctx.x_folded, ctas=1)
-            bsink = grad_sink(a[2])
-            db_a = bsink[0] if bsink is not None else torch.empty(4 * Ha, **f32)
-            dw_ha = _accumulate_grad(a[1], dg_a.t(), h_seq_a[:T].reshape(T * B, Ha), ctas=1,
-                                     rowsum=(db_a, bsink is not None and bsink[1]))
-            STATS["fused_bias_grads"] = STATS.get("fused_bias_grads", 0) + 1
-            if bsink is not None:
-                db_a = None
-                _grads_written()
-        else:
             dw_xa = _accumulate_grad(a[0], dg_a.t(), x2d, b_folded=ctx.x_folded)
             _bias_grad(a[2], dg_a, under_gemm=dw_xa is None, part=0)
             dw_ha = _accumulate_grad(a[1], dg_a.t(), h_seq_a[:T].reshape(T * B, Ha))
```
